# soasme/LTX-Video-GPUPoor

Measured on AMD Instinct MI355X. Metric: denoise-steps/sec + VAE-decode frames/sec, LTX-Video 768x512x97f at 1/8 GPU, higher is better.
Workload: dtype bf16

## Files before the change

include/ltxmi.h:

```cpp
#ifndef LTXMI_H
#define LTXMI_H

#include <stddef.h>
#include <stdint.h>

#ifdef __cplusplus
extern "C" {
#endif

typedef enum ltxmi_status {
    LTXMI_OK = 0,
    LTXMI_ERR_INVALID_ARG = -1,
    LTXMI_ERR_UNSUPPORTED = -2,
    LTXMI_ERR_LAUNCH = -3
} ltxmi_status;

const char* ltxmi_version(void);
const char* ltxmi_last_error(void);
const char* ltxmi_arch(void);

typedef enum ltxmi_epilogue {
    LTXMI_EPI_NONE = 0,
    LTXMI_EPI_GELU_TANH = 1,
    LTXMI_EPI_SILU = 2,
    LTXMI_EPI_GATE_RESIDUAL = 3
} ltxmi_epilogue;

typedef struct ltxmi_gemm_args {
    const void* A;  int64_t lda;
    const void* W;  int64_t ldw;
    const void* bias;
    void*       C;  int64_t ldc;
    int32_t M, N, K;
    int32_t epilogue;
    const void* residual; int64_t ldr;
    const void* gate_table;
    const void* gate_temb;
    int64_t     gate_ld;
    int32_t     rows_per_group;
    int32_t     algo;
    float*      rowsumsq; int32_t rowsumsq_cols; int64_t rowsumsq_ld;
    int32_t     a_kblock; int64_t a_kblock_stride;
} ltxmi_gemm_args;

int ltxmi_gemm_bf16(const ltxmi_gemm_args* args, void* stream);

typedef enum ltxmi_norm_kind { LTXMI_NORM_RMS = 0, LTXMI_NORM_LAYER = 1 } ltxmi_norm_kind;

int ltxmi_norm_modulate_bf16(const void* x, int64_t ldx, void* y, int64_t ldy,
                             int32_t rows, int32_t D, float eps, int32_t kind,
                             const void* scale_table, const void* scale_temb,
                             const void* shift_table, const void* shift_temb,
                             int64_t temb_ld, int32_t rows_per_group, void* stream);

int ltxmi_rmsnorm_rope_bf16(void* x, int64_t ldx, int32_t rows, int32_t D,
                            const void* weight, float eps,
                            const void* cos_tab, const void* sin_tab, int64_t ld_tab,
                            int32_t rope_period, void* stream);
int ltxmi_rmsnorm_rope_rstd_bf16(void* x, int64_t ldx, int32_t rows, int32_t D, const void* weight, float eps,
                                 const void* cos_tab, const void* sin_tab, int64_t ld_tab, int32_t rope_period,
                                 const float* rowsumsq, int64_t rowsumsq_ld, int32_t rowsumsq_blocks,
                                 int32_t norm_dim, float norm_eps, float* rstd_out, void* stream);

typedef struct ltxmi_attn_args {
    const void* q; int64_t q_stride_b, q_stride_l;
    const void* k; int64_t k_stride_b, k_stride_l;
    const void* v; int64_t v_stride_b, v_stride_l;
    void*       o; int64_t o_stride_b, o_stride_l;
    const float* key_bias; int64_t bias_stride_b;
    int32_t B, H, Lq, Lk, head_dim;
    float   softmax_scale;
    const float* q_rowsumsq; int64_t q_rowsumsq_stride_b, q_rowsumsq_stride_l; int32_t q_rowsumsq_blocks;
    const void*  q_norm_weight; float q_norm_eps;
    const void*  rope_cos; const void* rope_sin; int64_t rope_stride_b, rope_stride_l;
    int32_t o_segment_len; int64_t o_stride_segment;
    const float* q_rstd; int64_t q_rstd_stride_b, q_rstd_stride_l;
    uint32_t* redo_counter; int32_t force_exact;
    float* lse; int64_t lse_stride_b, lse_stride_h;
} ltxmi_attn_args;

int ltxmi_attention_fwd_bf16(const ltxmi_attn_args* args, void* stream);
int ltxmi_attention_fuses_qnorm(int32_t B, int32_t H, int32_t Lq, int32_t Lk, int32_t head_dim, int32_t has_key_bias);
int ltxmi_attention_kernel_id(int32_t B, int32_t H, int32_t Lq, int32_t Lk, int32_t head_dim, int32_t has_key_bias,
                              int64_t k_stride_l, int64_t v_stride_l);

#define LTXMI_ATTN_MERGE_MAX 8
typedef struct ltxmi_attn_merge_args {
    int32_t n;
    const void*  o_part[LTXMI_ATTN_MERGE_MAX];   int64_t o_part_stride_b[LTXMI_ATTN_MERGE_MAX], o_part_stride_l[LTXMI_ATTN_MERGE_MAX];
    const float* lse_part[LTXMI_ATTN_MERGE_MAX]; int64_t lse_part_stride_b[LTXMI_ATTN_MERGE_MAX], lse_part_stride_h[LTXMI_ATTN_MERGE_MAX];
    void*  o;   int64_t o_stride_b, o_stride_l;
    float* lse; int64_t lse_stride_b, lse_stride_h;
    int32_t B, H, Lq, head_dim;
} ltxmi_attn_merge_args;
int ltxmi_attention_merge_bf16(const ltxmi_attn_merge_args* args, void* stream);

int ltxmi_rowsumsq_rstd_f32(const float* rowsumsq, int64_t rowsumsq_ld, int32_t rowsumsq_blocks, int32_t rows,
                            int32_t norm_dim, float norm_eps, float* rstd_out, void* stream);

int ltxmi_qkv_norm_rope_pack_bf16(const void* qkv, int64_t ld, int32_t B, int32_t Nl, int32_t D, int32_t P,
                                  const void* q_weight, const void* k_weight, float eps, const void* cos_tab,
                                  const void* sin_tab, int64_t ld_tab, int32_t rope_period, void* out, void* stream);

int ltxmi_silu_bf16(const void* x, void* y, int64_t n, void* stream);
int ltxmi_timestep_embedding_bf16(const float* t, void* out, int32_t n, int32_t dim, void* stream);
int ltxmi_stg_blend_bf16(void* a, int64_t lda, const void* v, int64_t ldv,
                         const float* m, int32_t B, int32_t L, int32_t D, void* stream);
int ltxmi_stg_blend_grouped_bf16(void* a, const void* v, int64_t v_stride_g, int64_t v_stride_b, int64_t v_stride_l,
                                 const float* m, int32_t G, int32_t B, int32_t L, int32_t D, void* stream);

typedef struct ltxmi_conv3d_args {
    const void* x; const void* w; const void* bias; void* y;
    int32_t B, T, H, W, Cin, Cout;
    int32_t causal;
    int32_t pad_replicate;
    int32_t d2s;
    const void* residual;
    int32_t res_channels;
    const void* add;
    int32_t stride_t, stride_hw;
    int32_t tpad, out_T;
    int32_t kernel_t, time_pad_zeros;
    int32_t algo;
    int32_t post_norm;
    const float* post_scale;
    const float* post_shift;
    float post_eps;
    void* y_norm;
    void* workspace; int64_t workspace_bytes;
} ltxmi_conv3d_args;

int ltxmi_conv3d_ndhwc_bf16(const ltxmi_conv3d_args* args, void* stream);
int ltxmi_conv3d_fuses_post_norm(const ltxmi_conv3d_args* args);
int64_t ltxmi_conv3d_workspace_bytes(const ltxmi_conv3d_args* args);

int ltxmi_pixelnorm_ada_silu_bf16(const void* x, void* y, int64_t rows, int32_t C,
                                  int64_t rows_per_batch, const float* scale, const float* shift,
                                  int32_t apply_silu, float eps, void* stream);

int ltxmi_add_bf16(const void* a, const void* b, void* y, int64_t n, void* stream);

int ltxmi_layernorm_affine_bf16(const void* x, void* y, int64_t rows, int32_t C,
                                const void* gamma, const void* beta, float eps, void* stream);

int ltxmi_ncdhw_to_ndhwc_bf16(const void* z, void* y, int32_t B, int32_t C, int32_t T, int32_t H,
                              int32_t W, const float* std, const float* mean, void* stream);
int ltxmi_unpatchify_to_ncdhw_bf16(const void* x, void* y, int32_t B, int32_t T, int32_t H, int32_t W,
                                   int32_t C_out, int32_t patch, void* stream);

int ltxmi_patchify_to_ndhwc_bf16(const void* x, void* y, int32_t B, int32_t C, int32_t T, int32_t H,
                                 int32_t W, int32_t patch, int32_t C_pad, void* stream);
int ltxmi_space_to_depth_skip_bf16(const void* conv, const void* x, void* out, int32_t B, int32_t T,
                                   int32_t H, int32_t W, int32_t Cin, int32_t Cconv, int32_t stride_t,
                                   int32_t stride_hw, int32_t group, void* stream);
int ltxmi_ndhwc_to_ncdhw_bf16(const void* x, int64_t ldx, int32_t c0, void* y, int32_t B, int32_t C,
                              int32_t T, int32_t H, int32_t W, const float* std, const float* mean,
                              void* stream);

#define LTXMI_GUIDANCE_WORKSPACE_FLOATS 2048
int ltxmi_guidance_step_bf16(const void* noise_pred, int64_t n, int32_t num_conds,
                             float guidance_scale, float stg_scale, float rescaling_scale,
                             int32_t do_cfg, int32_t do_stg, int32_t do_rescale,
                             void* latents, int32_t latents_bf16, float dt, float* workspace,
                             void* stream);

int ltxmi_guidance_step_masked_bf16(const void* noise_pred, int64_t n, int32_t num_conds,
                                    float guidance_scale, float stg_scale, float rescaling_scale,
                                    int32_t do_cfg, int32_t do_stg, int32_t do_rescale,
                                    void* latents, int32_t latents_bf16, float dt,
                                    const float* cond_mask, int32_t channels, float t,
                                    float* workspace, void* stream);

int ltxmi_image_cond_noise(void* latents, const void* init_latents, const void* noise, int32_t is_bf16,
                           const float* cond_mask, int64_t tokens, int32_t channels, float noise_scale,
                           float t, void* stream);

int ltxmi_groupnorm_silu_bf16(const void* x, void* y, const void* residual, int32_t samples, int64_t S,
                              int32_t C, int32_t groups, const void* gamma, const void* beta, float eps,
                              float* workspace, void* stream);
int ltxmi_pixel_shuffle2d_ndhwc_bf16(const void* x, void* y, int64_t frames, int32_t H, int32_t W, int32_t C,
                                     void* stream);
int ltxmi_tile_blend(const void* a, void* b, int32_t dtype, int64_t outer, int64_t len_a, int64_t len_b,
                     int64_t inner, int32_t extent, void* stream);
int ltxmi_adain_filter(const void* latents, const void* reference, void* out, int32_t is_bf16, int32_t planes,
                       int64_t n, int64_t n_ref, float factor, void* stream);

#ifdef __cplusplus
}
#endif
#endif
```

ltx-video-gpupoor_amd/csrc/api.hip:

```cpp
#include <stdarg.h>
#include <string.h>

#include "common.h"

namespace ltxmi {

static thread_local char g_err[512] = "";

void set_error(const char* fmt, ...) {
    va_list ap;
    va_start(ap, fmt);
    vsnprintf(g_err, sizeof(g_err), fmt, ap);
    va_end(ap);
}

int check_launch(const char* what) {
    const hipError_t e = hipGetLastError();
    if (e != hipSuccess) {
        set_error("%s: launch failed: %s", what, hipGetErrorString(e));
        return LTXMI_ERR_LAUNCH;
    }
    return LTXMI_OK;
}

int reserve_lds(const void* kernel, int bytes, unsigned long long* done, const char* what) {
    int dev = 0;
    if (hipGetDevice(&dev) != hipSuccess) {
        set_error("%s: cannot query the current device", what);
        return LTXMI_ERR_LAUNCH;
    }
    const bool tracked = dev >= 0 && dev < 64;
    const unsigned long long bit = tracked ? (1ull << dev) : 0ull;
    if (tracked && (__atomic_load_n(done, __ATOMIC_ACQUIRE) & bit)) return LTXMI_OK;
    const hipError_t e = hipFuncSetAttribute(kernel, hipFuncAttributeMaxDynamicSharedMemorySize, bytes);
    if (e != hipSuccess) {
        set_error("%s: cannot reserve %d bytes of LDS: %s", what, bytes, hipGetErrorString(e));
        return LTXMI_ERR_LAUNCH;
    }
    if (tracked) __atomic_fetch_or(done, bit, __ATOMIC_RELEASE);
    return LTXMI_OK;
}

int device_cu_count(const char* what) {
    static int cus[64] = {};
    int dev = 0;
    if (hipGetDevice(&dev) != hipSuccess) {
        set_error("%s: cannot query the current device", what);
        return -1;
    }
    const bool tracked = dev >= 0 && dev < 64;
    if (tracked) {
        const int c = __atomic_load_n(&cus[dev], __ATOMIC_ACQUIRE);
        if (c > 0) return c;
    }
    int n = 0;
    if (hipDeviceGetAttribute(&n, hipDeviceAttributeMultiprocessorCount, dev) != hipSuccess || n <= 0) {
        set_error("%s: cannot query the CU count of device %d", what, dev);
        return -1;
    }
    if (tracked) __atomic_store_n(&cus[dev], n, __ATOMIC_RELEASE);
    return n;
}

}

extern "C" const char* ltxmi_version(void) { return "ltxmi 0.6.0 (round 5)"; }
extern "C" const char* ltxmi_last_error(void) { return ltxmi::g_err; }
extern "C" const char* ltxmi_arch(void) { return "gfx950"; }
```

ltx-video-gpupoor_amd/csrc/attention.h:

```cpp
#pragma once
#include "common.h"

namespace ltxmi {

struct AttnParams {
    const uint16_t* q; int64_t q_sb, q_sl;
    const uint16_t* k; int64_t k_sb, k_sl;
    const uint16_t* v; int64_t v_sb, v_sl;
    uint16_t* o; int64_t o_sb, o_sl;
    const float* bias; int64_t bias_sb;
    int B, H, Lq, Lk;
    float scale_log2e;
    int q_tiles;
    const float* q_ss; int64_t q_ss_sb, q_ss_sl; int q_ss_n;
    const float* q_rstd; int64_t q_rstd_sb, q_rstd_sl;
    const uint16_t* q_w; float q_eps;
    const uint16_t* rope_cos; const uint16_t* rope_sin; int64_t rope_sb, rope_sl;
    int o_seg; int64_t o_sseg;
    uint32_t* redo_count; int force_exact;
    float* lse; int64_t lse_sb, lse_sh;

    __host__ __device__ __forceinline__ bool q_on_load() const { return q_ss != nullptr || q_rstd != nullptr; }
    __device__ __forceinline__ float q_row_rstd(int b, int row, int HD) const {
        if (q_rstd) return q_rstd[(int64_t)b * q_rstd_sb + (int64_t)row * q_rstd_sl];
        const float* ss = q_ss + (int64_t)b * q_ss_sb + (int64_t)row * q_ss_sl;
        float s2 = 0.f;
        if ((q_ss_n & 3) == 0 && (((uintptr_t)ss) & 15) == 0) {
            const f32x4* ss4 = (const f32x4*)ss;
            for (int j = 0; j < (q_ss_n >> 2); ++j) {
                const f32x4 v4 = ss4[j];
                s2 += (v4[0] + v4[1]) + (v4[2] + v4[3]);
            }
        } else {
            for (int j = 0; j < q_ss_n; ++j) s2 += ss[j];
        }
        return rsqrtf(s2 / (float)HD + q_eps);
    }

    __device__ __forceinline__ void store_lse(int b, int head, int row, float m_log2, float l, bool removed) const {
        constexpr float LN2 = 0.6931471805599453f;
        lse[(int64_t)b * lse_sb + (int64_t)head * lse_sh + row] = removed ? -INFINITY : (m_log2 + __log2f(l)) * LN2;
    }

    __device__ __forceinline__ int64_t o_row(int row) const {
        if (o_seg <= 0) return (int64_t)row * o_sl;
        const int sg = row / o_seg;
        return (int64_t)sg * o_sseg + (int64_t)(row - sg * o_seg) * o_sl;
    }
};

enum AttnKernel : int {
    ATTN_DH64 = 0, ATTN_DH64_BIAS = 1, ATTN_DH64_QB2 = 2, ATTN_PIPE = 3,
    ATTN_DH128 = 4, ATTN_DH128_BIAS = 5, ATTN_PIPE128 = 6, ATTN_CROSS = 7,
};
constexpr int ATTN_CROSS_MAX_KEYS = 256;
constexpr float ATTN_BIAS_FLOOR = -1e30f;
constexpr float ATTN_ROW_REMOVED = 0.99f * ATTN_BIAS_FLOOR;

int launch_attn_pipe(AttnParams p, hipStream_t stream);
int launch_attn_pipe128(AttnParams p, hipStream_t stream);
int launch_attn_cross(AttnParams p, hipStream_t stream);

}
```

ltx-video-gpupoor_amd/csrc/attention.hip:

```cpp
#include <type_traits>

#include "attention.h"

namespace ltxmi {

constexpr int KV_TILE = 64;
constexpr int Q_PER_WAVE = 32;
constexpr int Q_PER_WG = 128;
constexpr float LOG2E = 1.4426950408889634f;
constexpr int ATTN_QB_BIG = 2;

template <int DH>
struct AttnCfg {
    static constexpr int ROW_BYTES = DH * 2;
    static constexpr int TILE_BYTES = KV_TILE * DH * 2;
    static constexpr int CHUNKS_PER_ROW = DH / 8;
    static constexpr int LD_PER_THREAD = (KV_TILE * CHUNKS_PER_ROW) / 256;
    static constexpr int KSTEPS = DH / 16;
    static constexpr int DBLK = DH / 32;
    static constexpr int BIAS_BYTES = KV_TILE * 4;
    static constexpr int STAGE_BYTES = 2 * TILE_BYTES + BIAS_BYTES;
    static constexpr int SMEM = 2 * STAGE_BYTES;
    __device__ static __forceinline__ int k_swz(int row) {
        return DH == 64 ? ((row >> 1) & 7) : (row & 15);
    }
};


template <int DH, bool HAS_BIAS, int QB>
__global__ __launch_bounds__(256, (QB == 2 || DH == 128) ? 2 : 1) void attn_fwd_kernel(AttnParams p) {
    using C = AttnCfg<DH>;
    constexpr int QW = Q_PER_WAVE * QB;
    constexpr bool FOLD = !HAS_BIAS && DH == 128;
    extern __shared__ __attribute__((aligned(16))) char smem[];

    const int tid = threadIdx.x;
    const int lane = tid & 63;
    const int wave = __builtin_amdgcn_readfirstlane(tid >> 6);
    const int r = lane & 31;
    const int hh = lane >> 5;

    const int nwg = gridDim.x, orig = blockIdx.x;
    const int xcd = orig & 7, qn = nwg >> 3, rn = nwg & 7;
    const int work = (xcd < rn ? xcd * (qn + 1) : rn * (qn + 1) + (xcd - rn) * qn) + (orig >> 3);
    const int bh = work / p.q_tiles, qt = work % p.q_tiles;
    const int b = bh / p.H, head = bh % p.H;

    const uint16_t* qb = p.q + (int64_t)b * p.q_sb + head * DH;
    const uint16_t* kb_ = p.k + (int64_t)b * p.k_sb + head * DH;
    const uint16_t* vb = p.v + (int64_t)b * p.v_sb + head * DH;
    uint16_t* ob = p.o + (int64_t)b * p.o_sb + head * DH;
    const float* biasb = HAS_BIAS ? p.bias + (int64_t)b * p.bias_sb : nullptr;

    int q_row[QB];
    bf16x8 qf[QB][C::KSTEPS];
#pragma unroll
    for (int i = 0; i < QB; ++i) {
        q_row[i] = qt * (4 * QW) + wave * QW + 32 * i + r;
        const int q_ld = q_row[i] < p.Lq ? q_row[i] : p.Lq - 1;
        const float rstd = p.q_on_load() ? p.q_row_rstd(b, q_ld, p.H * DH) : 0.f;
#pragma unroll
        for (int s = 0; s < C::KSTEPS; ++s) {
            qf[i][s] = *(const bf16x8*)(qb + (int64_t)q_ld * p.q_sl + 16 * s + 8 * hh);
            if (p.q_on_load()) {
                const int col = head * DH + 16 * s + 8 * hh;
                const bf16x8 wv = *(const bf16x8*)(p.q_w + col);
                float o[8];
#pragma unroll
                for (int e = 0; e < 8; ++e) o[e] = (float)qf[i][s][e] * rstd * (float)wv[e];
                if (p.rope_cos) {
                    const int64_t trow = (int64_t)b * p.rope_sb + (int64_t)q_ld * p.rope_sl;
                    const bf16x8 cv = *(const bf16x8*)(p.rope_cos + trow + col), sv = *(const bf16x8*)(p.rope_sin + trow + col);
#pragma unroll
                    for (int e = 0; e < 8; e += 2) {
                        const float r0 = o[e] * (float)cv[e] - o[e + 1] * (float)sv[e];
                        const float r1 = o[e + 1] * (float)cv[e + 1] + o[e] * (float)sv[e + 1];
                        o[e] = r0;
                        o[e + 1] = r1;
                    }
                }
#pragma unroll
                for (int e = 0; e < 8; ++e) qf[i][s][e] = (__bf16)o[e];
            }
            if (FOLD) {
#pragma unroll
                for (int e = 0; e < 8; ++e) qf[i][s][e] = (__bf16)((float)qf[i][s][e] * p.scale_log2e);
            }
        }
    }

    int st_key[C::LD_PER_THREAD], st_koff[C::LD_PER_THREAD], st_voff[C::LD_PER_THREAD], st_col[C::LD_PER_THREAD];
#pragma unroll
    for (int i = 0; i < C::LD_PER_THREAD; ++i) {
        const int c = tid + 256 * i;
        const int key = c / C::CHUNKS_PER_ROW, dc = c % C::CHUNKS_PER_ROW;
        st_key[i] = key;
        st_col[i] = dc * 8;
        st_koff[i] = key * C::ROW_BYTES + ((dc ^ C::k_swz(key)) << 4);
        st_voff[i] = C::TILE_BYTES + ((key >> 3) * C::DBLK + (dc >> 2)) * 512 + (key & 7) * 64 + (dc & 3) * 16;
    }
    u32x4 kreg[C::LD_PER_THREAD], vreg[C::LD_PER_THREAD];
    float breg = 0.f;

    uint32_t k_goff[C::LD_PER_THREAD], v_goff[C::LD_PER_THREAD];
#pragma unroll
    for (int i = 0; i < C::LD_PER_THREAD; ++i) {
        k_goff[i] = (uint32_t)(((int64_t)st_key[i] * p.k_sl + st_col[i]) * 2);
        v_goff[i] = (uint32_t)(((int64_t)st_key[i] * p.v_sl + st_col[i]) * 2);
    }
    auto load_tile = [&](int k0, auto tail_tag) {
        constexpr bool TAIL = decltype(tail_tag)::value;
        if (!TAIL) {
            const char* kt = (const char*)(kb_ + (int64_t)k0 * p.k_sl);
            const char* vt = (const char*)(vb + (int64_t)k0 * p.v_sl);
#pragma unroll
            for (int i = 0; i < C::LD_PER_THREAD; ++i) {
                kreg[i] = *(const u32x4*)(kt + k_goff[i]);
                vreg[i] = *(const u32x4*)(vt + v_goff[i]);
            }
        } else {
#pragma unroll
            for (int i = 0; i < C::LD_PER_THREAD; ++i) {
                int key = k0 + st_key[i];
                key = key < p.Lk ? key : p.Lk - 1;
                kreg[i] = *(const u32x4*)(kb_ + (int64_t)key * p.k_sl + st_col[i]);
                vreg[i] = *(const u32x4*)(vb + (int64_t)key * p.v_sl + st_col[i]);
            }
        }
        if (HAS_BIAS && tid < KV_TILE) {
            const int key = k0 + tid;
            breg = key < p.Lk ? fmaxf(biasb[key] * LOG2E, ATTN_BIAS_FLOOR) : 0.f;
        }
    };
    auto write_tile = [&](int buf) {
        char* s = smem + buf * C::STAGE_BYTES;
#pragma unroll
        for (int i = 0; i < C::LD_PER_THREAD; ++i) {
            *(u32x4*)(s + st_koff[i]) = kreg[i];
            *(u32x4*)(s + st_voff[i]) = vreg[i];
        }
        if (HAS_BIAS && tid < KV_TILE) *(float*)(s + 2 * C::TILE_BYTES + tid * 4) = breg;
    };

    int k_rd[2];
#pragma unroll
    for (int kb = 0; kb < 2; ++kb) k_rd[kb] = (32 * kb + r) * C::ROW_BYTES;
    const int k_sw0 = C::k_swz(r);
    const int g16 = lane >> 4, i16 = lane & 15;
    const int v_rd = C::TILE_BYTES + (4 * (g16 >> 1) + (i16 >> 2)) * 64 + (16 * (g16 & 1) + 4 * (i16 & 3)) * 2;

    f32x16 oT[QB][C::DBLK];
    float m_run[QB];
    f32x4 lT[QB];
    bf16x8 ones;
    {
        const bool on = ((lane & 15) == 0 && ((lane >> 4) & 1) == 0) || ((lane & 15) == 1 && ((lane >> 4) & 1) == 1);
#pragma unroll
        for (int e = 0; e < 8; ++e) ones[e] = on ? (__bf16)1.0f : (__bf16)0.0f;
    }
    bf16x8 kaug, maug[QB];
#pragma unroll
    for (int e = 0; e < 8; ++e) kaug[e] = (hh == 0 && e < 2) ? (__bf16)1.0f : (__bf16)0.0f;
#pragma unroll
    for (int i = 0; i < QB; ++i) {
        m_run[i] = FOLD ? 0.f : -INFINITY;
#pragma unroll
        for (int e = 0; e < 8; ++e) maug[i][e] = (__bf16)0.0f;
        lT[i] = f32x4{0.f, 0.f, 0.f, 0.f};
#pragma unroll
        for (int d = 0; d < C::DBLK; ++d)
#pragma unroll
            for (int e = 0; e < 16; ++e) oT[i][d][e] = 0.f;
    }
    const float c = p.scale_log2e;

    const int nt = (p.Lk + KV_TILE - 1) / KV_TILE;
    const int n_full = p.Lk / KV_TILE;

    auto tile_body = [&](int t, auto tail_tag) {
        constexpr bool TAIL = decltype(tail_tag)::value;
        const int cur = t & 1;
        const char* s = smem + cur * C::STAGE_BYTES;

        f32x16 sT[QB][2];
#pragma unroll
        for (int i = 0; i < QB; ++i)
#pragma unroll
            for (int kb = 0; kb < 2; ++kb) {
#pragma unroll
                for (int e = 0; e < 16; ++e) sT[i][kb][e] = 0.f;
                if (FOLD) sT[i][kb] = __builtin_amdgcn_mfma_f32_32x32x16_bf16(kaug, maug[i], sT[i][kb], 0, 0, 0);
#pragma unroll
                for (int ks = 0; ks < C::KSTEPS; ++ks) {
                    const bf16x8 kf = *(const bf16x8*)(s + k_rd[kb] + (((2 * ks + hh) ^ k_sw0) << 4));
                    sT[i][kb] = __builtin_amdgcn_mfma_f32_32x32x16_bf16(kf, qf[i][ks], sT[i][kb], 0, 0, 0);
                }
            }

#pragma unroll
        for (int i = 0; i < QB; ++i) {
            if (HAS_BIAS) {
                const float* bl = (const float*)(s + 2 * C::TILE_BYTES);
#pragma unroll
                for (int kb = 0; kb < 2; ++kb)
#pragma unroll
                    for (int g = 0; g < 4; ++g) {
                        const f32x4 b4 = *(const f32x4*)(bl + 32 * kb + 8 * g + 4 * hh);
#pragma unroll
                        for (int e = 0; e < 4; ++e)
                            sT[i][kb][4 * g + e] = __builtin_fmaf(sT[i][kb][4 * g + e], c, b4[e]);
                    }
            }
            if (TAIL) {
                const int k0 = t * KV_TILE;
#pragma unroll
                for (int kb = 0; kb < 2; ++kb)
#pragma unroll
                    for (int e = 0; e < 16; ++e) {
                        const int key = k0 + 32 * kb + (e & 3) + 8 * (e >> 2) + 4 * hh;
                        if (key >= p.Lk) sT[i][kb][e] = -INFINITY;
                    }
            }
            float mt;
            {
                auto max3 = [](float a, float b, float c3) { return fmaxf(fmaxf(a, b), c3); };
                float l1[11];
#pragma unroll
                for (int g = 0; g < 5; ++g) {
                    l1[g] = max3(sT[i][0][3 * g], sT[i][0][3 * g + 1], sT[i][0][3 * g + 2]);
                    l1[5 + g] = max3(sT[i][1][3 * g], sT[i][1][3 * g + 1], sT[i][1][3 * g + 2]);
                }
                l1[10] = max3(sT[i][0][15], sT[i][1][15], l1[0]);
                const float a = max3(l1[1], l1[2], l1[3]), b2 = max3(l1[4], l1[5], l1[6]), c2 = max3(l1[7], l1[8], l1[9]);
                mt = fmaxf(max3(a, b2, c2), l1[10]);
            }
            {
                const auto sw = __builtin_amdgcn_permlane32_swap(__float_as_uint(mt), __float_as_uint(mt), false, false);
                mt = fmaxf(__uint_as_float(sw[0]), __uint_as_float(sw[1]));
            }
            float nmoff = 0.f;
            if (FOLD) {
                const bool first = (t == 0);
                if (first || __any(mt > 0.f)) {
                    asm volatile("; max-moved branch (kept a real branch: not if-converted)" ::: "memory");
                    const float dq = (first || mt > 0.f) ? ceilf(mt * 4.0f) * 0.25f : 0.f;
#pragma unroll
                    for (int kb = 0; kb < 2; ++kb)
#pragma unroll
                        for (int e = 0; e < 16; ++e) sT[i][kb][e] -= dq;
                    if (!first) {
                        const float alpha = fast_exp2(-dq);
                        lT[i][0] *= alpha;
                        lT[i][1] *= __shfl(alpha, (lane + 16) & 63, 64);
#pragma unroll
                        for (int d = 0; d < C::DBLK; ++d)
#pragma unroll
                            for (int e = 0; e < 16; ++e) oT[i][d][e] *= alpha;
                    }
                    m_run[i] += dq;
                    const float nm = -m_run[i];
                    const __bf16 mh = (__bf16)nm;
                    const __bf16 ml = (__bf16)(nm - (float)mh);
                    maug[i][0] = hh == 0 ? mh : (__bf16)0.0f;
                    maug[i][1] = hh == 0 ? ml : (__bf16)0.0f;
                }
            } else {
                const float m_new = fmaxf(m_run[i], mt);
                if (__any(m_new != m_run[i])) {
                    asm volatile("; rescale branch (kept a real branch: not if-converted)" ::: "memory");
                    const float alpha = HAS_BIAS ? fast_exp2(m_run[i] - m_new) : fast_exp2((m_run[i] - m_new) * c);
                    lT[i][0] *= alpha;
                    lT[i][1] *= __shfl(alpha, (lane + 16) & 63, 64);
#pragma unroll
                    for (int d = 0; d < C::DBLK; ++d)
#pragma unroll
                        for (int e = 0; e < 16; ++e) oT[i][d][e] *= alpha;
                    m_run[i] = m_new;
                }
                nmoff = HAS_BIAS ? -m_run[i] : -m_run[i] * c;
            }

            bf16x8 pf[4];
#pragma unroll
            for (int kb = 0; kb < 2; ++kb) {
#pragma unroll
                for (int e = 0; e < 16; ++e) {
                    sT[i][kb][e] = fast_exp2(FOLD ? sT[i][kb][e] : (HAS_BIAS ? sT[i][kb][e] + nmoff : __builtin_fmaf(sT[i][kb][e], c, nmoff)));
                }
#pragma unroll
                for (int h2 = 0; h2 < 2; ++h2)
#pragma unroll
                    for (int e = 0; e < 8; ++e) pf[2 * kb + h2][e] = (__bf16)sT[i][kb][8 * h2 + e];
            }

#pragma unroll
            for (int sp = 0; sp < 4; ++sp) {
                lT[i] = __builtin_amdgcn_mfma_f32_16x16x32_bf16(ones, pf[sp], lT[i], 0, 0, 0);
#pragma unroll
                for (int d = 0; d < C::DBLK; ++d) {
                    const char* base = s + v_rd + (2 * sp * C::DBLK + d) * 512;
                    const s16x4 lo = __builtin_amdgcn_ds_read_tr16_b64_v4i16(
                        (__attribute__((address_space(3))) s16x4*)(base));
                    const s16x4 hi = __builtin_amdgcn_ds_read_tr16_b64_v4i16(
                        (__attribute__((address_space(3))) s16x4*)(base + C::DBLK * 512));
                    typedef __attribute__((ext_vector_type(8))) short s16x8;
                    const s16x8 both = __builtin_shufflevector(lo, hi, 0, 1, 2, 3, 4, 5, 6, 7);
                    const bf16x8 vf = __builtin_bit_cast(bf16x8, both);
                    oT[i][d] = __builtin_amdgcn_mfma_f32_32x32x16_bf16(vf, pf[sp], oT[i][d], 0, 0, 0);
                }
            }
        }
    };

    using no_tail = std::integral_constant<bool, false>;
    using with_tail = std::integral_constant<bool, true>;
    if (n_full > 0) load_tile(0, no_tail{}); else load_tile(0, with_tail{});
    write_tile(0);
    __syncthreads();

    for (int t = 0; t < n_full; ++t) {
        const bool has_next = t + 1 < nt;
        if (has_next) {
            if (t + 1 < n_full) load_tile((t + 1) * KV_TILE, no_tail{});
            else load_tile((t + 1) * KV_TILE, with_tail{});
        }
        tile_body(t, no_tail{});
        if (has_next) write_tile((t & 1) ^ 1);
        __syncthreads();
    }
    if (n_full < nt) tile_body(n_full, with_tail{});

#pragma unroll
    for (int i = 0; i < QB; ++i) {
        const float l0 = __shfl(lT[i][0], r & 15, 64), l1 = __shfl(lT[i][1], r & 15, 64);
        const float l = (r & 16) ? l1 : l0;
        const float inv = 1.0f / l;
        if (p.lse != nullptr) {
            const float m2 = (HAS_BIAS || FOLD) ? m_run[i] : m_run[i] * c;
            if (hh == 0 && q_row[i] < p.Lq) p.store_lse(b, head, q_row[i], m2, l, HAS_BIAS && m_run[i] <= ATTN_ROW_REMOVED);
        }
        char* scr = smem + wave * (32 * C::ROW_BYTES);
        if (i == 0) __syncthreads();
#pragma unroll
        for (int d = 0; d < C::DBLK; ++d)
#pragma unroll
            for (int g = 0; g < 4; ++g) {
                u32x2 w;
                w[0] = pack_bf16(oT[i][d][4 * g + 0] * inv, oT[i][d][4 * g + 1] * inv);
                w[1] = pack_bf16(oT[i][d][4 * g + 2] * inv, oT[i][d][4 * g + 3] * inv);
                const int chunk = 4 * d + g;
                *(u32x2*)(scr + r * C::ROW_BYTES + ((chunk ^ (r & 7)) << 4) + hh * 8) = w;
            }
        constexpr int LPR = C::CHUNKS_PER_ROW;
        constexpr int RPI = 64 / LPR;
        const int q0 = qt * (4 * QW) + wave * QW + 32 * i;
#pragma unroll
        for (int t = 0; t < 32 / RPI; ++t) {
            const int row = t * RPI + lane / LPR, chunk = lane % LPR;
            const u32x4 w = *(const u32x4*)(scr + row * C::ROW_BYTES + ((chunk ^ (row & 7)) << 4));
            if (q0 + row < p.Lq) *(u32x4*)(ob + p.o_row(q0 + row) + chunk * 8) = w;
        }
    }
}

template <int DH, bool HAS_BIAS, int QB>
static int launch(AttnParams p, hipStream_t stream) {
    using C = AttnCfg<DH>;
    auto kern = attn_fwd_kernel<DH, HAS_BIAS, QB>;
    static unsigned long long lds_done = 0;
    if (const int rc = reserve_lds((const void*)kern, C::SMEM, &lds_done, "ltxmi_attention_fwd_bf16")) return rc;
    const int q_per_wg = Q_PER_WG * QB;
    p.q_tiles = (p.Lq + q_per_wg - 1) / q_per_wg;
    const int64_t grid = (int64_t)p.B * p.H * p.q_tiles;
    hipLaunchKernelGGL(kern, dim3((unsigned)grid), dim3(256), C::SMEM, stream, p);
    return check_launch("ltxmi_attention_fwd_bf16");
}

static AttnKernel attn_select(int B, int H, int Lq, int Lk, int head_dim, bool has_bias, int64_t k_sl, int64_t v_sl) {
    const int64_t wg256 = (int64_t)B * H * ((Lq + 255) / 256);
    const int64_t rows = (int64_t)Lk + 4 * 64;
    const bool span_ok = (rows * k_sl + head_dim) * 2 < (1ll << 31) && (rows * v_sl + head_dim) * 2 < (1ll << 31);
    if (head_dim == 128) {
        if (!has_bias && wg256 >= 128 && Lk >= 1024 && span_ok) return ATTN_PIPE128;
        return has_bias ? ATTN_DH128_BIAS : ATTN_DH128;
    }
    if (Lk <= ATTN_CROSS_MAX_KEYS && Lq >= 1024) return ATTN_CROSS;
    if (!has_bias && wg256 >= 192 && span_ok) return ATTN_PIPE;
    if (!has_bias && wg256 >= 512) return ATTN_DH64_QB2;
    return has_bias ? ATTN_DH64_BIAS : ATTN_DH64;
}

}

using namespace ltxmi;

extern "C" int ltxmi_attention_fwd_bf16(const ltxmi_attn_args* a, void* stream) {
    LTXMI_REQUIRE(a && a->q && a->k && a->v && a->o, LTXMI_ERR_INVALID_ARG, "ltxmi_attention_fwd_bf16: NULL argument");
    LTXMI_REQUIRE(a->B > 0 && a->H > 0 && a->Lq > 0 && a->Lk > 0, LTXMI_ERR_INVALID_ARG,
                  "ltxmi_attention_fwd_bf16: non-positive shape B=%d H=%d Lq=%d Lk=%d", a->B, a->H, a->Lq, a->Lk);
    LTXMI_REQUIRE(a->head_dim == 64 || a->head_dim == 128, LTXMI_ERR_UNSUPPORTED,
                  "ltxmi_attention_fwd_bf16: head_dim %d not in {64, 128}", a->head_dim);
    const int64_t strides[] = {a->q_stride_b, a->q_stride_l, a->k_stride_b, a->k_stride_l,
                               a->v_stride_b, a->v_stride_l, a->o_stride_b, a->o_stride_l};
    for (int64_t s : strides)
        LTXMI_REQUIRE(s % 8 == 0, LTXMI_ERR_UNSUPPORTED, "ltxmi_attention_fwd_bf16: strides must be multiples of 8 elements");
    LTXMI_REQUIRE((((uintptr_t)a->q | (uintptr_t)a->k | (uintptr_t)a->v | (uintptr_t)a->o) & 15) == 0,
                  LTXMI_ERR_UNSUPPORTED, "ltxmi_attention_fwd_bf16: q/k/v/o must be 16-byte aligned");
    LTXMI_REQUIRE((int64_t)a->B * a->H * ((a->Lq + Q_PER_WG - 1) / Q_PER_WG) < (1ll << 31), LTXMI_ERR_UNSUPPORTED,
                  "ltxmi_attention_fwd_bf16: grid too large");
    AttnParams p;
    p.q = (const uint16_t*)a->q; p.q_sb = a->q_stride_b; p.q_sl = a->q_stride_l;
    p.k = (const uint16_t*)a->k; p.k_sb = a->k_stride_b; p.k_sl = a->k_stride_l;
    p.v = (const uint16_t*)a->v; p.v_sb = a->v_stride_b; p.v_sl = a->v_stride_l;
    p.o = (uint16_t*)a->o; p.o_sb = a->o_stride_b; p.o_sl = a->o_stride_l;
    p.bias = a->key_bias; p.bias_sb = a->bias_stride_b;
    p.B = a->B; p.H = a->H; p.Lq = a->Lq; p.Lk = a->Lk;
    p.scale_log2e = a->softmax_scale * LOG2E;
    p.q_tiles = (a->Lq + Q_PER_WG - 1) / Q_PER_WG;
    p.q_ss = a->q_rowsumsq; p.q_ss_sb = a->q_rowsumsq_stride_b; p.q_ss_sl = a->q_rowsumsq_stride_l;
    p.q_ss_n = a->q_rowsumsq_blocks;
    p.q_rstd = a->q_rstd; p.q_rstd_sb = a->q_rstd_stride_b; p.q_rstd_sl = a->q_rstd_stride_l;
    p.q_w = (const uint16_t*)a->q_norm_weight; p.q_eps = a->q_norm_eps;
    p.rope_cos = (const uint16_t*)a->rope_cos; p.rope_sin = (const uint16_t*)a->rope_sin;
    p.rope_sb = a->rope_stride_b; p.rope_sl = a->rope_stride_l;
    p.o_seg = a->o_segment_len; p.o_sseg = a->o_stride_segment;
    p.redo_count = a->redo_counter; p.force_exact = a->force_exact != 0;
    LTXMI_REQUIRE(a->o_segment_len >= 0 && a->o_stride_segment % 8 == 0, LTXMI_ERR_INVALID_ARG,
                  "ltxmi_attention_fwd_bf16: bad output segment geometry");
    p.lse = a->lse; p.lse_sb = a->lse_stride_b; p.lse_sh = a->lse_stride_h;
    if (a->lse)
        LTXMI_REQUIRE((((uintptr_t)a->lse) & 3) == 0 && a->lse_stride_h >= a->Lq &&
                          (a->B == 1 ? a->lse_stride_b >= 0 : a->lse_stride_b >= (int64_t)a->H * a->lse_stride_h),
                      LTXMI_ERR_INVALID_ARG,
                      "ltxmi_attention_fwd_bf16: lse must be 4-byte aligned with lse_stride_h >= Lq and lse_stride_b >= H * lse_stride_h");
    if (a->q_rowsumsq || a->q_rstd) {
        LTXMI_REQUIRE(a->q_norm_weight && (((uintptr_t)a->q_norm_weight) & 15) == 0 &&
                          (a->q_rstd ? (((uintptr_t)a->q_rstd) & 3) == 0
                                     : (a->q_rowsumsq_blocks == a->H * a->head_dim / 64 && (((uintptr_t)a->q_rowsumsq) & 3) == 0)),
                      LTXMI_ERR_INVALID_ARG, "ltxmi_attention_fwd_bf16: bad q_rowsumsq / q_rstd / q_norm_weight geometry");
        LTXMI_REQUIRE((a->rope_cos == nullptr) == (a->rope_sin == nullptr), LTXMI_ERR_INVALID_ARG,
                      "ltxmi_attention_fwd_bf16: rope_cos and rope_sin must both be given or both be NULL");
        if (a->rope_cos)
            LTXMI_REQUIRE((((uintptr_t)a->rope_cos | (uintptr_t)a->rope_sin) & 15) == 0 && a->rope_stride_l % 8 == 0 &&
                              a->rope_stride_b % 8 == 0,
                          LTXMI_ERR_INVALID_ARG, "ltxmi_attention_fwd_bf16: RoPE tables must be 16-byte aligned rows");
    }
    hipStream_t s = (hipStream_t)stream;
    switch (attn_select(a->B, a->H, a->Lq, a->Lk, a->head_dim, a->key_bias != nullptr, a->k_stride_l, a->v_stride_l)) {
        case ATTN_DH64: return launch<64, false, 1>(p, s);
        case ATTN_DH64_BIAS: return launch<64, true, 1>(p, s);
        case ATTN_DH64_QB2: return launch<64, false, ATTN_QB_BIG>(p, s);
        case ATTN_PIPE: return launch_attn_pipe(p, s);
        case ATTN_DH128: return launch<128, false, 1>(p, s);
        case ATTN_DH128_BIAS: return launch<128, true, 1>(p, s);
        case ATTN_PIPE128: return launch_attn_pipe128(p, s);
        case ATTN_CROSS: return launch_attn_cross(p, s);
    }
}

extern "C" int ltxmi_attention_kernel_id(int32_t B, int32_t H, int32_t Lq, int32_t Lk, int32_t head_dim, int32_t has_key_bias,
                                         int64_t k_stride_l, int64_t v_stride_l) {
    if (B <= 0 || H <= 0 || Lq <= 0 || Lk <= 0 || k_stride_l <= 0 || v_stride_l <= 0) return -1;
    if (head_dim != 64 && head_dim != 128) return -1;
    return attn_select(B, H, Lq, Lk, head_dim, has_key_bias != 0, k_stride_l, v_stride_l);
}

extern "C" int ltxmi_attention_fuses_qnorm(int32_t B, int32_t H, int32_t Lq, int32_t Lk, int32_t head_dim, int32_t has_key_bias) {
    return (B > 0 && H > 0 && Lq > 0 && Lk > 0 && (head_dim == 64 || head_dim == 128) && (H * head_dim) % 64 == 0) ? 1 : 0;
}
```

ltx-video-gpupoor_amd/csrc/attention_cross.hip:

```cpp
#include <type_traits>

#include "attention.h"

namespace ltxmi {

namespace cross {

#ifndef LTXMI_XATTN_STAGGER
#define LTXMI_XATTN_STAGGER 32
#endif

constexpr int DH = 64;
constexpr int KV_TILE = 64;
constexpr int MAX_TILES = 4;
constexpr int ROW_BYTES = DH * 2;
constexpr int TILE_BYTES = KV_TILE * DH * 2;
constexpr int K_OFF = 0, V_OFF = MAX_TILES * TILE_BYTES, BIAS_OFF = 2 * MAX_TILES * TILE_BYTES;
constexpr int SCR_OFF = BIAS_OFF + MAX_TILES * KV_TILE * 16;
constexpr int SCR_BYTES = 32 * 64;
constexpr int QW_OFF = SCR_OFF + 4 * SCR_BYTES;
constexpr int SMEM = QW_OFF + DH * 2;
constexpr int ROWS_PER_IT = 128;
constexpr float LOG2E = 1.4426950408889634f;

__device__ __forceinline__ int k_swz(int row) { return (row >> 1) & 7; }

template <int NT>
__global__ __launch_bounds__(256, 2) void attn_cross_kernel(AttnParams p, int groups, int rows_per_group, int stagger_from) {
    extern __shared__ __attribute__((aligned(16))) char smem[];
    const int tid = threadIdx.x;
    const int lane = tid & 63;
    const int wave = __builtin_amdgcn_readfirstlane(tid >> 6);
    const int r = lane & 31, hh = lane >> 5;

    const int nwg = gridDim.x, orig = blockIdx.x;
    const int xcd = orig & 7, qn = nwg >> 3, rn = nwg & 7;
    const int work = (xcd < rn ? xcd * (qn + 1) : rn * (qn + 1) + (xcd - rn) * qn) + (orig >> 3);
    const int bh = work / groups, grp = work % groups;
    const int b = bh / p.H, head = bh % p.H;
    const int row_begin = grp * rows_per_group;
    const int row_end = min(p.Lq, row_begin + rows_per_group);
    if (row_begin >= row_end) return;
    const int n_it = (row_end - row_begin + ROWS_PER_IT - 1) / ROWS_PER_IT;

    const uint16_t* qb = p.q + (int64_t)b * p.q_sb + head * DH;
    const uint16_t* kb_ = p.k + (int64_t)b * p.k_sb + head * DH;
    const uint16_t* vb = p.v + (int64_t)b * p.v_sb + head * DH;
    uint16_t* ob = p.o + (int64_t)b * p.o_sb + head * DH;
    constexpr int nt = NT;

    {
        u32x4 kreg[NT][2], vreg[NT][2];
#pragma unroll
        for (int t = 0; t < NT; ++t) {
#pragma unroll
                for (int i = 0; i < 2; ++i) {
                    const int c = tid + 256 * i;
                    int key = t * KV_TILE + (c >> 3);
                    key = key < p.Lk ? key : p.Lk - 1;
                    kreg[t][i] = *(const u32x4*)(kb_ + (int64_t)key * p.k_sl + (c & 7) * 8);
                    vreg[t][i] = *(const u32x4*)(vb + (int64_t)key * p.v_sl + (c & 7) * 8);
                }
            }
        if (tid < MAX_TILES * KV_TILE) {
            float bv = ATTN_BIAS_FLOOR;
            if (tid < p.Lk) bv = p.bias ? fmaxf(p.bias[(int64_t)b * p.bias_sb + tid] * (LOG2E / p.scale_log2e), ATTN_BIAS_FLOOR) : 0.f;
            const __bf16 hi = (__bf16)bv;
            const __bf16 lo = (__bf16)(bv - (float)hi);
            u32x4 w = {0u, 0u, 0u, 0u};
            w[0] = (uint32_t)__builtin_bit_cast(uint16_t, hi) | ((uint32_t)__builtin_bit_cast(uint16_t, lo) << 16);
            *(u32x4*)(smem + BIAS_OFF + tid * 16) = w;
        }
#pragma unroll
        for (int t = 0; t < NT; ++t) {
#pragma unroll
                for (int i = 0; i < 2; ++i) {
                    const int c = tid + 256 * i;
                    const int key = c >> 3, dc = c & 7;
                    *(u32x4*)(smem + K_OFF + t * TILE_BYTES + key * ROW_BYTES + ((dc ^ k_swz(key)) << 4)) = kreg[t][i];
                    *(u32x4*)(smem + V_OFF + t * TILE_BYTES + ((key >> 3) * 2 + (dc >> 2)) * 512 + (key & 7) * 64 + (dc & 3) * 16) = vreg[t][i];
                }
            }
    }
    if (p.q_on_load() && tid < 8) *(u32x4*)(smem + QW_OFF + tid * 16) = *(const u32x4*)(p.q_w + head * DH + tid * 8);
    __syncthreads();

    const int k_rd0 = r * ROW_BYTES, k_rd1 = (32 + r) * ROW_BYTES;
    const int k_sw0 = k_swz(r);
    const int g16 = lane >> 4, i16 = lane & 15;
    const int v_rd = (4 * (g16 >> 1) + (i16 >> 2)) * 64 + (16 * (g16 & 1) + 4 * (i16 & 3)) * 2;
    bf16x8 ones;
    {
        const bool on = ((lane & 15) == 0 && ((lane >> 4) & 1) == 0) || ((lane & 15) == 1 && ((lane >> 4) & 1) == 1);
#pragma unroll
        for (int e = 0; e < 8; ++e) ones[e] = on ? (__bf16)1.0f : (__bf16)0.0f;
    }
    const float c = p.scale_log2e;
    char* scr = smem + SCR_OFF + wave * SCR_BYTES;

    bf16x8 qraw[4], qf[4];
    float q_rstd = 0.f;
    int q_ld = 0;
    auto load_q = [&](int it) {
        const int row = row_begin + it * ROWS_PER_IT + wave * 32 + r;
        q_ld = row < p.Lq ? row : p.Lq - 1;
#pragma unroll
        for (int s = 0; s < 4; ++s) qraw[s] = *(const bf16x8*)(qb + (int64_t)q_ld * p.q_sl + 16 * s + 8 * hh);
        if (p.q_on_load()) q_rstd = p.q_row_rstd(b, q_ld, p.H * DH);
    };
    auto finish_q = [&]() {
        if (p.q_on_load()) {
            const int64_t trow = (int64_t)b * p.rope_sb + (int64_t)q_ld * p.rope_sl;
#pragma unroll
            for (int s = 0; s < 4; ++s) {
                const bf16x8 wv = *(const bf16x8*)(smem + QW_OFF + (16 * s + 8 * hh) * 2);
                float o[8];
#pragma unroll
                for (int e = 0; e < 8; ++e) o[e] = (float)qraw[s][e] * q_rstd * (float)wv[e];
                if (p.rope_cos) {
                    const int col = head * DH + 16 * s + 8 * hh;
                    const bf16x8 cv = *(const bf16x8*)(p.rope_cos + trow + col), sv = *(const bf16x8*)(p.rope_sin + trow + col);
#pragma unroll
                    for (int e = 0; e < 8; e += 2) {
                        const float r0 = o[e] * (float)cv[e] - o[e + 1] * (float)sv[e];
                        const float r1 = o[e + 1] * (float)cv[e + 1] + o[e] * (float)sv[e + 1];
                        o[e] = r0;
                        o[e + 1] = r1;
                    }
                }
#pragma unroll
                for (int e = 0; e < 8; ++e) qf[s][e] = (__bf16)o[e];
            }
        } else {
#pragma unroll
            for (int s = 0; s < 4; ++s) qf[s] = qraw[s];
        }
    };
    load_q(0);
    finish_q();
    if (n_it > 1) load_q(1);
    if (blockIdx.x >= (unsigned)stagger_from) __builtin_amdgcn_s_sleep(LTXMI_XATTN_STAGGER);

    for (int it = 0; it < n_it; ++it) {
        const int q0 = row_begin + it * ROWS_PER_IT + wave * 32;

        constexpr int NG = 2 * NT;
        f32x16 sT[NG];
        bf16x8 kfr[5];
        bf16x8 qaug;
        {
            uint32_t w0 = hh == 0 ? 0x3f803f80u : 0u, w1 = 0u;
            asm volatile("" : "+v"(w0), "+v"(w1));
            const u32x4 w = {w0, w1, w1, w1};
            qaug = __builtin_bit_cast(bf16x8, w);
        }
        auto read_k1 = [&](int g, int j) {
            if (j == 0) {
                kfr[0] = *(const bf16x8*)(smem + BIAS_OFF + (32 * g + r) * 16);
            } else {
                const char* ks = smem + K_OFF + (g >> 1) * TILE_BYTES + ((g & 1) ? k_rd1 : k_rd0);
                kfr[j] = *(const bf16x8*)(ks + (((2 * (j - 1) + hh) ^ k_sw0) << 4));
            }
        };
        auto max3 = [](float a, float b2, float c3) { return fmaxf(fmaxf(a, b2), c3); };
        float mt = -INFINITY;
        auto group_max = [&](int g) {
            const f32x16& x = sT[g];
            const float a = max3(x[0], x[1], x[2]), b2 = max3(x[3], x[4], x[5]), c2 = max3(x[6], x[7], x[8]);
            const float d2 = max3(x[9], x[10], x[11]), e2 = max3(x[12], x[13], x[14]);
            mt = max3(max3(a, b2, c2), max3(d2, e2, x[15]), mt);
            asm volatile("" : "+v"(mt));
        };
#pragma unroll
        for (int j = 0; j < 5; ++j) read_k1(0, j);
#pragma unroll
        for (int g = 0; g < NG; ++g) {
#pragma unroll
            for (int j = 0; j < 5; ++j) {
                if (j == 0) {
                    const f32x16 z16 = {0.f, 0.f, 0.f, 0.f, 0.f, 0.f, 0.f, 0.f, 0.f, 0.f, 0.f, 0.f, 0.f, 0.f, 0.f, 0.f};
                    sT[g] = __builtin_amdgcn_mfma_f32_32x32x16_bf16(kfr[0], qaug, z16, 0, 0, 0);
                } else {
                    sT[g] = __builtin_amdgcn_mfma_f32_32x32x16_bf16(kfr[j], qf[j - 1], sT[g], 0, 0, 0);
                }
                if (g + 1 < NG) read_k1(g + 1, j);
                __builtin_amdgcn_sched_barrier(0);
            }
            if (g >= 1) group_max(g - 1);
        }
        if (it + 1 < n_it) finish_q();
        if (it + 2 < n_it) load_q(it + 2);
        group_max(NG - 1);
        {
            const auto sw = __builtin_amdgcn_permlane32_swap(__float_as_uint(mt), __float_as_uint(mt), false, false);
            mt = fmaxf(__uint_as_float(sw[0]), __uint_as_float(sw[1]));
        }
        const float nmc = -mt * c;

        f32x16 oT[2];
        f32x4 lT;
        const f32x16 z16 = {0.f, 0.f, 0.f, 0.f, 0.f, 0.f, 0.f, 0.f, 0.f, 0.f, 0.f, 0.f, 0.f, 0.f, 0.f, 0.f};
        const f32x4 z4 = {0.f, 0.f, 0.f, 0.f};
        typedef __attribute__((ext_vector_type(8))) short s16x8;
        auto read_v = [&](int t, int sp, bf16x8 (&dst)[2]) {
            const char* vs = smem + V_OFF + t * TILE_BYTES + v_rd;
#pragma unroll
            for (int d = 0; d < 2; ++d) {
                const char* base = vs + (2 * sp * 2 + d) * 512;
                const s16x4 lo = __builtin_amdgcn_ds_read_tr16_b64_v4i16((__attribute__((address_space(3))) s16x4*)(base));
                const s16x4 hi = __builtin_amdgcn_ds_read_tr16_b64_v4i16((__attribute__((address_space(3))) s16x4*)(base + 2 * 512));
                const s16x8 both = __builtin_shufflevector(lo, hi, 0, 1, 2, 3, 4, 5, 6, 7);
                dst[d] = __builtin_bit_cast(bf16x8, both);
            }
        };
        auto make_p = [&](int t, int sp2, bf16x8& dst) {
            const f32x16& x = sT[2 * t + (sp2 >> 1)];
            const f32x2 c2v = {c, c}, m2v = {nmc, nmc};
#pragma unroll
            for (int e = 0; e < 8; e += 2) {
                const f32x2 y = f32x2{x[8 * (sp2 & 1) + e], x[8 * (sp2 & 1) + e + 1]} * c2v + m2v;
                dst[e] = (__bf16)fast_exp2(y[0]);
                dst[e + 1] = (__bf16)fast_exp2(y[1]);
            }
            asm volatile("" : "+v"(dst));
        };
        bf16x8 pfr[2][4], vfr[2][2];
#pragma unroll
        for (int sp = 0; sp < 4; ++sp) make_p(0, sp, pfr[0][sp]);
        read_v(0, 0, vfr[0]);
#pragma unroll
        for (int t = 0; t < NT; ++t) {
#pragma unroll
            for (int sp = 0; sp < 4; ++sp) {
                const int st = 4 * t + sp;
                if (st + 1 < 4 * NT) read_v((st + 1) >> 2, (st + 1) & 3, vfr[(st + 1) & 1]);
                const bf16x8& pf = pfr[t & 1][sp];
                lT = __builtin_amdgcn_mfma_f32_16x16x32_bf16(ones, pf, st == 0 ? z4 : lT, 0, 0, 0);
                oT[0] = __builtin_amdgcn_mfma_f32_32x32x16_bf16(vfr[st & 1][0], pf, st == 0 ? z16 : oT[0], 0, 0, 0);
                oT[1] = __builtin_amdgcn_mfma_f32_32x32x16_bf16(vfr[st & 1][1], pf, st == 0 ? z16 : oT[1], 0, 0, 0);
                if (t + 1 < NT) make_p(t + 1, sp, pfr[(t + 1) & 1][sp]);
                __builtin_amdgcn_sched_barrier(0);
            }
        }

        const float l0 = __shfl(lT[0], r & 15, 64), l1v = __shfl(lT[1], r & 15, 64);
        const float lrow = (r & 16) ? l1v : l0;
        const float inv = 1.0f / lrow;
        if (p.lse != nullptr) {
            if (hh == 0 && q0 + r < row_end) p.store_lse(b, head, q0 + r, -nmc, lrow, -nmc / c <= ATTN_ROW_REMOVED);
        }
#pragma unroll
        for (int d = 0; d < 2; ++d) {
#pragma unroll
            for (int g = 0; g < 4; ++g) {
                u32x2 w;
                w[0] = pack_bf16(oT[d][4 * g + 0] * inv, oT[d][4 * g + 1] * inv);
                w[1] = pack_bf16(oT[d][4 * g + 2] * inv, oT[d][4 * g + 3] * inv);
                *(u32x2*)(scr + r * 64 + ((g ^ (r & 3)) << 4) + hh * 8) = w;
            }
#pragma unroll
            for (int t2 = 0; t2 < 2; ++t2) {
                const int row = t2 * 16 + (lane >> 2), chunk = lane & 3;
                const u32x4 w = *(const u32x4*)(scr + row * 64 + ((chunk ^ (row & 3)) << 4));
                if (q0 + row < row_end) *(u32x4*)(ob + p.o_row(q0 + row) + 32 * d + chunk * 8) = w;
            }
        }
    }
}

}

static_assert(cross::MAX_TILES * cross::KV_TILE == ATTN_CROSS_MAX_KEYS, "attn_select hands this kernel up to ATTN_CROSS_MAX_KEYS keys");

int launch_attn_cross(AttnParams p, hipStream_t stream) {
    const int n_cu = device_cu_count("ltxmi_attention_fwd_bf16");
    if (n_cu <= 0) return LTXMI_ERR_LAUNCH;
    const int slots = 2 * n_cu, bh = p.B * p.H;
    int groups = slots / bh;
    if (groups < 1) groups = 1;
    const int max_groups = (p.Lq + 2 * cross::ROWS_PER_IT - 1) / (2 * cross::ROWS_PER_IT);
    if (groups > max_groups) groups = max_groups;
    int rows = (p.Lq + groups - 1) / groups;
    rows = (rows + cross::ROWS_PER_IT - 1) / cross::ROWS_PER_IT * cross::ROWS_PER_IT;
    groups = (p.Lq + rows - 1) / rows;
    const int64_t grid = (int64_t)bh * groups;
    const int nt = (p.Lk + cross::KV_TILE - 1) / cross::KV_TILE;
#define LTXMI_XATTN_LAUNCH(N)                                                                                              \
    {                                                                                                                      \
        static unsigned long long lds_done = 0;                                                                            \
        if (const int rc = reserve_lds((const void*)cross::attn_cross_kernel<N>, cross::SMEM, &lds_done,                   \
                                       "ltxmi_attention_fwd_bf16"))                                                        \
            return rc;                                                                                                     \
        hipLaunchKernelGGL(cross::attn_cross_kernel<N>, dim3((unsigned)grid), dim3(256), cross::SMEM, stream, p, groups,   \
                           rows, n_cu);                                                                                    \
    }
    switch (nt) {
        case 1: LTXMI_XATTN_LAUNCH(1) break;
        case 2: LTXMI_XATTN_LAUNCH(2) break;
        case 3: LTXMI_XATTN_LAUNCH(3) break;
        default: LTXMI_XATTN_LAUNCH(4) break;
    }
#undef LTXMI_XATTN_LAUNCH
    return check_launch("ltxmi_attention_fwd_bf16");
}

}
```

ltx-video-gpupoor_amd/ltxmi/_lib.py:

```python
import ctypes
import os

import torch

_HERE = os.path.dirname(os.path.abspath(__file__))
LIB_PATH = os.environ.get("LTXMI_LIB") or os.path.join(_HERE, "libltxmi.so")

c_void_p, c_int, c_int64, c_float = ctypes.c_void_p, ctypes.c_int32, ctypes.c_int64, ctypes.c_float


class GemmArgs(ctypes.Structure):
    _fields_ = [("A", c_void_p), ("lda", c_int64), ("W", c_void_p), ("ldw", c_int64), ("bias", c_void_p),
                ("C", c_void_p), ("ldc", c_int64), ("M", c_int), ("N", c_int), ("K", c_int),
                ("epilogue", c_int), ("residual", c_void_p), ("ldr", c_int64), ("gate_table", c_void_p),
                ("gate_temb", c_void_p), ("gate_ld", c_int64), ("rows_per_group", c_int), ("algo", c_int),
                ("rowsumsq", c_void_p), ("rowsumsq_cols", c_int), ("rowsumsq_ld", c_int64),
                ("a_kblock", c_int), ("a_kblock_stride", c_int64)]


class AttnArgs(ctypes.Structure):
    _fields_ = [("q", c_void_p), ("q_stride_b", c_int64), ("q_stride_l", c_int64),
                ("k", c_void_p), ("k_stride_b", c_int64), ("k_stride_l", c_int64),
                ("v", c_void_p), ("v_stride_b", c_int64), ("v_stride_l", c_int64),
                ("o", c_void_p), ("o_stride_b", c_int64), ("o_stride_l", c_int64),
                ("key_bias", c_void_p), ("bias_stride_b", c_int64),
                ("B", c_int), ("H", c_int), ("Lq", c_int), ("Lk", c_int), ("head_dim", c_int),
                ("softmax_scale", c_float),
                ("q_rowsumsq", c_void_p), ("q_rowsumsq_stride_b", c_int64), ("q_rowsumsq_stride_l", c_int64),
                ("q_rowsumsq_blocks", c_int), ("q_norm_weight", c_void_p), ("q_norm_eps", c_float),
                ("rope_cos", c_void_p), ("rope_sin", c_void_p), ("rope_stride_b", c_int64), ("rope_stride_l", c_int64),
                ("o_segment_len", c_int), ("o_stride_segment", c_int64),
                ("q_rstd", c_void_p), ("q_rstd_stride_b", c_int64), ("q_rstd_stride_l", c_int64),
                ("redo_counter", c_void_p), ("force_exact", c_int),
                ("lse", c_void_p), ("lse_stride_b", c_int64), ("lse_stride_h", c_int64)]


ATTN_MERGE_MAX = 8


class AttnMergeArgs(ctypes.Structure):
    _fields_ = [("n", c_int),
                ("o_part", c_void_p * ATTN_MERGE_MAX), ("o_part_stride_b", c_int64 * ATTN_MERGE_MAX),
                ("o_part_stride_l", c_int64 * ATTN_MERGE_MAX),
                ("lse_part", c_void_p * ATTN_MERGE_MAX), ("lse_part_stride_b", c_int64 * ATTN_MERGE_MAX),
                ("lse_part_stride_h", c_int64 * ATTN_MERGE_MAX),
                ("o", c_void_p), ("o_stride_b", c_int64), ("o_stride_l", c_int64),
                ("lse", c_void_p), ("lse_stride_b", c_int64), ("lse_stride_h", c_int64),
                ("B", c_int), ("H", c_int), ("Lq", c_int), ("head_dim", c_int)]


class Conv3dArgs(ctypes.Structure):
    _fields_ = [("x", c_void_p), ("w", c_void_p), ("bias", c_void_p), ("y", c_void_p),
                ("B", c_int), ("T", c_int), ("H", c_int), ("W", c_int), ("Cin", c_int), ("Cout", c_int),
                ("causal", c_int), ("pad_replicate", c_int), ("d2s", c_int), ("residual", c_void_p),
                ("res_channels", c_int), ("add", c_void_p),
                ("stride_t", c_int), ("stride_hw", c_int), ("tpad", c_int), ("out_T", c_int),
                ("kernel_t", c_int), ("time_pad_zeros", c_int), ("algo", c_int),
                ("post_norm", c_int), ("post_scale", c_void_p), ("post_shift", c_void_p), ("post_eps", c_float),
                ("y_norm", c_void_p), ("workspace", c_void_p), ("workspace_bytes", c_int64)]


SIGNATURES = {
    "ltxmi_version": (ctypes.c_char_p, []),
    "ltxmi_last_error": (ctypes.c_char_p, []),
    "ltxmi_arch": (ctypes.c_char_p, []),
    "ltxmi_gemm_bf16": (c_int, [ctypes.POINTER(GemmArgs), c_void_p]),
    "ltxmi_norm_modulate_bf16": (c_int, [c_void_p, c_int64, c_void_p, c_int64, c_int, c_int, c_float, c_int,
                                         c_void_p, c_void_p, c_void_p, c_void_p, c_int64, c_int, c_void_p]),
    "ltxmi_rmsnorm_rope_bf16": (c_int, [c_void_p, c_int64, c_int, c_int, c_void_p, c_float, c_void_p, c_void_p,
                                        c_int64, c_int, c_void_p]),
    "ltxmi_rmsnorm_rope_rstd_bf16": (c_int, [c_void_p, c_int64, c_int, c_int, c_void_p, c_float, c_void_p, c_void_p,
                                             c_int64, c_int, c_void_p, c_int64, c_int, c_int, c_float, c_void_p, c_void_p]),
    "ltxmi_rowsumsq_rstd_f32": (c_int, [c_void_p, c_int64, c_int, c_int, c_int, c_float, c_void_p, c_void_p]),
    "ltxmi_qkv_norm_rope_pack_bf16": (c_int, [c_void_p, c_int64, c_int, c_int, c_int, c_int, c_void_p, c_void_p, c_float,
                                              c_void_p, c_void_p, c_int64, c_int, c_void_p, c_void_p]),
    "ltxmi_attention_fwd_bf16": (c_int, [ctypes.POINTER(AttnArgs), c_void_p]),
    "ltxmi_attention_merge_bf16": (c_int, [ctypes.POINTER(AttnMergeArgs), c_void_p]),
    "ltxmi_attention_fuses_qnorm": (c_int, [c_int, c_int, c_int, c_int, c_int, c_int]),
    "ltxmi_attention_kernel_id": (c_int, [c_int, c_int, c_int, c_int, c_int, c_int, c_int64, c_int64]),
    "ltxmi_silu_bf16": (c_int, [c_void_p, c_void_p, c_int64, c_void_p]),
    "ltxmi_timestep_embedding_bf16": (c_int, [c_void_p, c_void_p, c_int, c_int, c_void_p]),
    "ltxmi_stg_blend_bf16": (c_int, [c_void_p, c_int64, c_void_p, c_int64, c_void_p, c_int, c_int, c_int, c_void_p]),
    "ltxmi_stg_blend_grouped_bf16": (c_int, [c_void_p, c_void_p, c_int64, c_int64, c_int64, c_void_p, c_int, c_int, c_int, c_int,
                                             c_void_p]),
    "ltxmi_conv3d_ndhwc_bf16": (c_int, [ctypes.POINTER(Conv3dArgs), c_void_p]),
    "ltxmi_conv3d_fuses_post_norm": (c_int, [ctypes.POINTER(Conv3dArgs)]),
    "ltxmi_conv3d_workspace_bytes": (c_int64, [ctypes.POINTER(Conv3dArgs)]),
    "ltxmi_pixelnorm_ada_silu_bf16": (c_int, [c_void_p, c_void_p, c_int64, c_int, c_int64, c_void_p, c_void_p,
                                              c_int, c_float, c_void_p]),
    "ltxmi_add_bf16": (c_int, [c_void_p, c_void_p, c_void_p, c_int64, c_void_p]),
    "ltxmi_layernorm_affine_bf16": (c_int, [c_void_p, c_void_p, c_int64, c_int, c_void_p, c_void_p, c_float,
                                            c_void_p]),
    "ltxmi_ncdhw_to_ndhwc_bf16": (c_int, [c_void_p, c_void_p, c_int, c_int, c_int, c_int, c_int, c_void_p,
                                          c_void_p, c_void_p]),
    "ltxmi_unpatchify_to_ncdhw_bf16": (c_int, [c_void_p, c_void_p, c_int, c_int, c_int, c_int, c_int, c_int,
                                               c_void_p]),
    "ltxmi_guidance_step_masked_bf16": (c_int, [c_void_p, c_int64, c_int, c_float, c_float, c_float, c_int, c_int,
                                                c_int, c_void_p, c_int, c_float, c_void_p, c_int, c_float, c_void_p,
                                                c_void_p]),
    "ltxmi_image_cond_noise": (c_int, [c_void_p, c_void_p, c_void_p, c_int, c_void_p, c_int64, c_int, c_float,
                                       c_float, c_void_p]),
    "ltxmi_groupnorm_silu_bf16": (c_int, [c_void_p, c_void_p, c_void_p, c_int, c_int64, c_int, c_int, c_void_p,
                                          c_void_p, c_float, c_void_p, c_void_p]),
    "ltxmi_pixel_shuffle2d_ndhwc_bf16": (c_int, [c_void_p, c_void_p, c_int64, c_int, c_int, c_int, c_void_p]),
    "ltxmi_adain_filter": (c_int, [c_void_p, c_void_p, c_void_p, c_int, c_int, c_int64, c_int64, c_float, c_void_p]),
    "ltxmi_tile_blend": (c_int, [c_void_p, c_void_p, c_int, c_int64, c_int64, c_int64, c_int64, c_int, c_void_p]),
    "ltxmi_patchify_to_ndhwc_bf16": (c_int, [c_void_p, c_void_p, c_int, c_int, c_int, c_int, c_int, c_int, c_int,
                                             c_void_p]),
    "ltxmi_space_to_depth_skip_bf16": (c_int, [c_void_p, c_void_p, c_void_p, c_int, c_int, c_int, c_int, c_int,
                                               c_int, c_int, c_int, c_int, c_void_p]),
    "ltxmi_ndhwc_to_ncdhw_bf16": (c_int, [c_void_p, c_int64, c_int, c_void_p, c_int, c_int, c_int, c_int, c_int,
                                          c_void_p, c_void_p, c_void_p]),
    "ltxmi_guidance_step_bf16": (c_int, [c_void_p, c_int64, c_int, c_float, c_float, c_float, c_int, c_int, c_int,
                                         c_void_p, c_int, c_float, c_void_p, c_void_p]),
}


def _load():
    if not os.path.exists(LIB_PATH):
        raise ImportError(
            f"ltxmi: {LIB_PATH} is missing -- build it with `make -C ltx-video-gpupoor_amd/csrc` "
            "(or `python -c 'import __graft_entry__ as g; g.build()'`). There is no fallback path.")
    lib = ctypes.CDLL(LIB_PATH)
    for name, (res, args) in SIGNATURES.items():
        fn = getattr(lib, name)
        fn.restype = res
        fn.argtypes = args
    return lib


lib = _load()


class LtxmiError(RuntimeError):
    pass


def check(status, what):
    if status != 0:
        raise LtxmiError(f"{what} failed ({status}): {lib.ltxmi_last_error().decode()}")
```

ltx-video-gpupoor_amd/ltxmi/attention.py:

```python
from enum import Enum, auto
from typing import Optional

import torch
from torch import nn

from . import ops
from .attention_seam import pay_attention

BF16 = torch.bfloat16


FUSE_CROSS_ATTENTION_Q = True


class SkipLayerStrategy(Enum):
    AttentionSkip = auto()
    AttentionValues = auto()
    Residual = auto()
    TransformerBlock = auto()


def reshape_hidden_states(hidden_states, latent_frames):
    return hidden_states.reshape(hidden_states.shape[0], latent_frames, -1, hidden_states.shape[-1])


def restore_hidden_states_shape(hidden_states):
    return hidden_states.reshape(hidden_states.shape[0], -1, hidden_states.shape[-1])


class RMSNorm(nn.Module):

    def __init__(self, dim, eps: float, elementwise_affine: bool = True):
        super().__init__()
        self.eps = eps
        self.dim = dim
        if elementwise_affine:
            self.weight = nn.Parameter(torch.ones(dim))
        else:
            self.register_parameter("weight", None)


class _NoAffineLayerNorm(nn.Module):
    def __init__(self, dim, eps: float, elementwise_affine: bool = False):
        super().__init__()
        if elementwise_affine:
            raise NotImplementedError("ltxmi: standardisation norms with affine parameters are not on this path")
        self.eps = eps
        self.dim = dim


class GELUProj(nn.Module):

    def __init__(self, dim_in, dim_out, approximate="tanh", bias=True):
        super().__init__()
        self.proj = nn.Linear(dim_in, dim_out, bias=bias)
        self.approximate = approximate


class FeedForward(nn.Module):

    def __init__(self, dim, dim_out=None, mult=4, dropout=0.0, activation_fn="geglu", final_dropout=False,
                 inner_dim=None, bias=True):
        super().__init__()
        if activation_fn != "gelu-approximate":
            raise NotImplementedError(f"ltxmi: activation_fn '{activation_fn}' is not on this path "
                                      "(LTX-Video uses 'gelu-approximate')")
        inner_dim = int(dim * mult) if inner_dim is None else inner_dim
        dim_out = dim if dim_out is None else dim_out
        self.net = nn.ModuleList([GELUProj(dim, inner_dim, "tanh", bias), nn.Dropout(dropout),
                                  nn.Linear(inner_dim, dim_out, bias=bias)])

    def forward(self, hidden_states, scale: float = 1.0):
        h = ops.gemm(hidden_states, self.net[0].proj.weight, self.net[0].proj.bias, epilogue=ops.EPI_GELU_TANH)
        out = ops.gemm(h, self.net[2].weight, self.net[2].bias)
        return out.view(*hidden_states.shape[:-1], out.shape[-1])


class Attention(nn.Module):

    def __init__(self, query_dim, cross_attention_dim=None, heads=8, dim_head=64, dropout=0.0, bias=False,
                 upcast_attention=False, upcast_softmax=False, out_bias=True, scale_qk=True, qk_norm=None,
                 eps=1e-5, rescale_output_factor=1.0, residual_connection=False, processor=None, out_dim=None,
                 use_tpu_flash_attention=False, use_rope=False, **unsupported):
        super().__init__()
        for k, v in unsupported.items():
            if v not in (None, False, 32):
                raise NotImplementedError(f"ltxmi.Attention: argument {k}={v} is not on this path")
        if use_tpu_flash_attention:
            raise NotImplementedError("ltxmi.Attention: TPU flash attention does not exist on MI355X")
        self.inner_dim = out_dim if out_dim is not None else dim_head * heads
        self.query_dim = query_dim
        self.use_bias = bias
        self.is_cross_attention = cross_attention_dim is not None
        self.cross_attention_dim = cross_attention_dim if cross_attention_dim is not None else query_dim
        self.rescale_output_factor = rescale_output_factor
        self.residual_connection = residual_connection
        self.out_dim = out_dim if out_dim is not None else query_dim
        self.use_tpu_flash_attention = False
        self.use_rope = use_rope
        self.scale = dim_head ** -0.5 if scale_qk else 1.0
        self.heads = out_dim // dim_head if out_dim is not None else heads
        if qk_norm is None:
            self.q_norm, self.k_norm = nn.Identity(), nn.Identity()
        elif qk_norm == "rms_norm":
            self.q_norm = RMSNorm(dim_head * heads, eps=1e-5)
            self.k_norm = RMSNorm(dim_head * heads, eps=1e-5)
        else:
            raise NotImplementedError(f"ltxmi.Attention: qk_norm '{qk_norm}' is not on this path")
        self.to_q = nn.Linear(query_dim, self.inner_dim, bias=bias)
        self.to_k = nn.Linear(self.cross_attention_dim, self.inner_dim, bias=bias)
        self.to_v = nn.Linear(self.cross_attention_dim, self.inner_dim, bias=bias)
        self.to_out = nn.ModuleList([nn.Linear(self.inner_dim, self.out_dim, bias=out_bias), nn.Dropout(dropout)])
        self._packs = {}
        self.set_processor(processor if processor is not None else AttnProcessor2_0())

    def set_processor(self, processor) -> None:
        self.processor = processor

    def get_processor(self, return_deprecated_lora: bool = False):
        return self.processor

    def _pack(self, slot, mods):
        srcs = [t for m in mods for t in (m.weight, m.bias) if t is not None]
        key = tuple((t.data_ptr(), ops.tensor_version(t), t.dtype, t.device) for t in srcs)
        hit = self._packs.get(slot)
        if hit is None or hit[0] != key:
            with torch.no_grad():
                w = torch.cat([m.weight for m in mods], dim=0).contiguous()
                b = torch.cat([m.bias for m in mods], dim=0).contiguous() if mods[0].bias is not None else None
            hit = (key, w, b)
            self._packs[slot] = hit
        return hit[1], hit[2]

    def packed_qkv(self):
        if self.cross_attention_dim != self.query_dim:
            raise ValueError("ltxmi.Attention.packed_qkv: query and key/value inputs differ")
        return self._pack("qkv", [self.to_q, self.to_k, self.to_v])

    def packed_kv(self):
        return self._pack("kv", [self.to_k, self.to_v])

    def invalidate_packed(self):
        self._packs = {}
        self.__dict__.pop("_text_kv_cache", None)

    def _load_from_state_dict(self, *a, **k):
        self.invalidate_packed()
        return super()._load_from_state_dict(*a, **k)

    def _apply(self, fn, *a, **k):
        self.invalidate_packed()
        return super()._apply(fn, *a, **k)

    def forward(self, hidden_states, freqs_cis=None, encoder_hidden_states=None, attention_mask=None,
                skip_layer_mask=None, skip_layer_strategy=None, fused_residual=None, **cross_attention_kwargs):
        wrapper = hidden_states if isinstance(hidden_states, list) else [hidden_states]
        return self.processor(self, wrapper, freqs_cis=freqs_cis, encoder_hidden_states=encoder_hidden_states,
                              attention_mask=attention_mask, skip_layer_mask=skip_layer_mask,
                              skip_layer_strategy=skip_layer_strategy, fused_residual=fused_residual)


def _host_mask(mask):
    if mask is None:
        return None
    host = getattr(mask, "_ltxmi_host", None)
    return host if host is not None else [float(x) for x in mask.flatten().tolist()]


class AttnProcessor2_0:

    def attend(self, qkv_list, is_cross, **kw):
        return pay_attention(qkv_list, **kw)

    def __call__(self, attn: Attention, hidden_states_wrapper, freqs_cis, encoder_hidden_states=None,
                 attention_mask=None, temb=None, skip_layer_mask=None, skip_layer_strategy=None,
                 fused_residual=None, *args, **kwargs):
        hidden_states = hidden_states_wrapper[0]
        hidden_states_wrapper.clear()
        if hidden_states.dim() != 3:
            raise NotImplementedError("ltxmi.AttnProcessor2_0: only [B, N, D] inputs are on this path")
        B, N, _ = hidden_states.shape
        D = attn.inner_dim
        H = attn.heads
        dh = D // H
        x2 = hidden_states.reshape(B * N, -1)
        is_cross = encoder_hidden_states is not None
        if is_cross:
            wkv, bkv = attn.packed_kv()
        else:
            wqkv, bqkv = attn.packed_qkv()
        if not isinstance(attn.q_norm, RMSNorm):
            raise NotImplementedError("ltxmi.AttnProcessor2_0: qk_norm=None is not on this path")

        q_fused = None
        if not is_cross:
            fuse_q = ops.attention_fuses_qnorm(B, H, N, N, dh) and D % 64 == 0 and attention_mask is None
            ss = torch.empty((B * N, D // 64), dtype=torch.float32, device=x2.device) if fuse_q else None
            qkv = ops.gemm(x2, wqkv, bqkv, rowsumsq=ss, rowsumsq_cols=D if fuse_q else 0)
            q2, k2, v2 = qkv[:, :D], qkv[:, D:2 * D], qkv[:, 2 * D:]
            cos = sin = None
            period = 0
            if attn.use_rope:
                cos, sin = freqs_cis
                if cos.shape[0] not in (1, B):
                    raise ValueError("freqs_cis batch must be 1 or the batch size")
                cos2, sin2 = cos.reshape(-1, D), sin.reshape(-1, D)
                period = cos2.shape[0]
                cos, sin = cos2, sin2
            if fuse_q:
                rstd = torch.empty((B * N,), dtype=torch.float32, device=x2.device)
                ops.rmsnorm_rope_(k2, attn.k_norm.weight, attn.k_norm.eps, cos, sin, period,
                                  rstd_of=(ss, D, attn.q_norm.eps, rstd))
                q_fused = ((rstd, attn.q_norm.weight, attn.q_norm.eps), (cos, sin, period) if cos is not None else None)
            else:
                ops.rmsnorm_rope_(q2, attn.q_norm.weight, attn.q_norm.eps, cos, sin, period)
                ops.rmsnorm_rope_(k2, attn.k_norm.weight, attn.k_norm.eps, cos, sin, period)
            Lk = N
            q4 = qkv.view(B, N, 3, H, dh)[:, :, 0]
            k4 = qkv.view(B, N, 3, H, dh)[:, :, 1]
            v4 = qkv.view(B, N, 3, H, dh)[:, :, 2]
            v3 = qkv.view(B, N, 3 * D)[:, :, 2 * D:]
        else:
            Bk, Lk, _ = encoder_hidden_states.shape
            fuse_q = FUSE_CROSS_ATTENTION_Q and D % 64 == 0 and bool(ops.attention_fuses_qnorm(B, H, N, Lk, dh, attention_mask is not None))
            ss = torch.empty((B * N, D // 64), dtype=torch.float32, device=x2.device) if fuse_q else None
            q2 = ops.gemm(x2, attn.to_q.weight, attn.to_q.bias, rowsumsq=ss, rowsumsq_cols=D if fuse_q else 0)
            ehs = encoder_hidden_states
            key = (ehs.data_ptr(), tuple(ehs.shape), ops.tensor_version(ehs), wkv.data_ptr(), ops.tensor_version(wkv),
                   attn.k_norm.weight.data_ptr(), ops.tensor_version(attn.k_norm.weight))
            cache = attn.__dict__.setdefault("_text_kv_cache", {})
            hit = cache.get(key) if ops.STEP_INVARIANT_CACHING else None
            if hit is None:
                ready = attn.__dict__.get("_text_kv_ready")
                if ready is not None:
                    full, full_version, kv_full = ready
                    row_bytes = full.stride(0) * full.element_size()
                    off = ehs.data_ptr() - full.data_ptr()
                    if (row_bytes > 0 and off >= 0 and off % row_bytes == 0 and ehs.shape[1:] == full.shape[1:]
                            and off // row_bytes + Bk <= full.shape[0] and ehs.dtype == full.dtype and ehs.is_contiguous()
                            and ops.tensor_version(full) == full_version):
                        r0 = off // row_bytes
                        hit = (kv_full[r0 * Lk:(r0 + Bk) * Lk],)
            if hit is None:
                kv = ops.gemm(ehs.reshape(Bk * Lk, -1), wkv, bkv)
                ops.rmsnorm_rope_(kv[:, :D], attn.k_norm.weight, attn.k_norm.eps)
                if len(cache) >= 4:
                    cache.clear()
                if ops.STEP_INVARIANT_CACHING:
                    cache[key] = (kv, ehs, wkv)
            else:
                kv = hit[0]
            if fuse_q:
                q_fused = ((ops.rowsumsq_rstd(ss, D, attn.q_norm.eps), attn.q_norm.weight, attn.q_norm.eps), None)
            else:
                ops.rmsnorm_rope_(q2, attn.q_norm.weight, attn.q_norm.eps)
            q4 = q2.view(B, N, H, dh)
            k4 = kv.view(Bk, Lk, 2, H, dh)[:, :, 0]
            v4 = kv.view(Bk, Lk, 2, H, dh)[:, :, 1]
            v3 = kv.view(Bk, Lk, 2 * D)[:, :, D:]

        host_mask = _host_mask(skip_layer_mask) if skip_layer_mask is not None else None
        skip_attention = (host_mask is not None and skip_layer_strategy == SkipLayerStrategy.AttentionValues
                          and len(host_mask) == 1 and host_mask[0] == 0)
        if skip_attention:
            a3 = v3.contiguous()
        else:
            mask4 = None
            if attention_mask is not None:
                if attention_mask.dim() != 3 or attention_mask.shape[1] != 1:
                    raise NotImplementedError("ltxmi.AttnProcessor2_0: attention_mask must be a [B,1,Lk] bias")
                mask4 = attention_mask.reshape(B, 1, 1, Lk)
            a4 = self.attend([q4, k4, v4], is_cross, attention_mask=mask4, softmax_scale=attn.scale,
                             q_norm=q_fused[0] if q_fused else None, rope=q_fused[1] if q_fused else None)
            a3 = a4.view(B, N, D)
            if host_mask is not None and any(m != 1.0 for m in host_mask):
                m_dev = skip_layer_mask.reshape(B).to(torch.float32)
                if skip_layer_strategy == SkipLayerStrategy.AttentionValues:
                    ops.stg_blend_(a3, v3, m_dev)
                elif skip_layer_strategy == SkipLayerStrategy.AttentionSkip:
                    ops.stg_blend_(a3, hidden_states, m_dev)

        w_o, b_o = attn.to_out[0].weight, attn.to_out[0].bias
        if fused_residual is not None:
            residual, gate_table, gate_temb, rpg = fused_residual
            ops.gemm(a3.reshape(B * N, D), w_o, b_o, out=residual.reshape(B * N, -1),
                     epilogue=ops.EPI_GATE_RESIDUAL, residual=residual.reshape(B * N, -1),
                     gate_table=gate_table, gate_temb=gate_temb, rows_per_group=rpg)
            return residual
        out = ops.gemm(a3.reshape(B * N, D), w_o, b_o).view(B, N, -1)
        if attn.residual_connection or attn.rescale_output_factor != 1.0:
            raise NotImplementedError("ltxmi.AttnProcessor2_0: residual_connection / rescale_output_factor")
        return out


class BasicTransformerBlock(nn.Module):

    def __init__(self, dim, num_attention_heads, attention_head_dim, dropout=0.0, cross_attention_dim=None,
                 activation_fn="geglu", num_embeds_ada_norm=None, attention_bias=False, only_cross_attention=False,
                 double_self_attention=False, upcast_attention=False, norm_elementwise_affine=True,
                 adaptive_norm="single_scale_shift", standardization_norm="layer_norm", norm_eps=1e-5,
                 qk_norm=None, final_dropout=False, attention_type="default", ff_inner_dim=None, ff_bias=True,
                 attention_out_bias=True, use_tpu_flash_attention=False, use_rope=False):
        super().__init__()
        if adaptive_norm != "single_scale_shift" or only_cross_attention or double_self_attention:
            raise NotImplementedError("ltxmi.BasicTransformerBlock: only the AdaLN-Zero "
                                      "(single_scale_shift) self+cross block is on this path")
        assert standardization_norm in ("layer_norm", "rms_norm")
        self.adaptive_norm = adaptive_norm
        self.norm_kind = ops.NORM_RMS if standardization_norm == "rms_norm" else ops.NORM_LAYER
        make_norm = RMSNorm if standardization_norm == "rms_norm" else _NoAffineLayerNorm
        if norm_elementwise_affine:
            raise NotImplementedError("ltxmi.BasicTransformerBlock: norm_elementwise_affine=True is not on this path")
        self.norm1 = make_norm(dim, eps=norm_eps, elementwise_affine=False)
        self.attn1 = Attention(query_dim=dim, heads=num_attention_heads, dim_head=attention_head_dim,
                               dropout=dropout, bias=attention_bias, cross_attention_dim=None,
                               out_bias=attention_out_bias, qk_norm=qk_norm, use_rope=use_rope)
        if cross_attention_dim is not None:
            self.attn2 = Attention(query_dim=dim, cross_attention_dim=cross_attention_dim,
                                   heads=num_attention_heads, dim_head=attention_head_dim, dropout=dropout,
                                   bias=attention_bias, out_bias=attention_out_bias, qk_norm=qk_norm,
                                   use_rope=use_rope)
        else:
            self.attn2 = None
        self.norm2 = make_norm(dim, norm_eps, False)
        self.ff = FeedForward(dim, dropout=dropout, activation_fn=activation_fn, final_dropout=final_dropout,
                              inner_dim=ff_inner_dim, bias=ff_bias)
        self.scale_shift_table = nn.Parameter(torch.randn(6, dim) / dim ** 0.5)

    def prepare_shared_state(self):
        self.attn1.packed_qkv()
        if self.attn2 is not None:
            self.attn2.packed_kv()

    def forward(self, hidden_states, freqs_cis=None, attention_mask=None, encoder_hidden_states=None,
                encoder_attention_mask=None, timestep=None, cross_attention_kwargs=None, class_labels=None,
                added_cond_kwargs=None, skip_layer_mask=None, skip_layer_strategy: Optional[SkipLayerStrategy] = None):
        if attention_mask is not None:
            raise NotImplementedError("ltxmi.BasicTransformerBlock: a self-attention mask is not on this path")
        B, N, D = hidden_states.shape
        assert timestep.ndim == 3
        T1 = timestep.shape[1]
        if N % T1 != 0:
            raise ValueError(f"per-frame modulation needs tokens ({N}) divisible by frames ({T1})")
        rpg = N // T1
        host_mask = _host_mask(skip_layer_mask)
        if host_mask is not None and min(host_mask) == 1.0:
            skip_layer_mask, host_mask = None, None
        table = self.scale_shift_table
        temb = timestep.reshape(B * T1, 6 * D)
        h2 = hidden_states.view(B * N, D)

        def chunk(i):
            return table[i], temb[:, i * D:(i + 1) * D]

        norm_h = torch.empty_like(hidden_states)
        sc_t, sc_e = chunk(1)
        sh_t, sh_e = chunk(0)
        ops.norm_modulate(h2, norm_h.view(B * N, D), self.norm1.eps, self.norm_kind, sc_t, sc_e, sh_t, sh_e, rpg)
        g_t, g_e = chunk(2)
        self.attn1([norm_h], freqs_cis=freqs_cis, skip_layer_mask=skip_layer_mask,
                   skip_layer_strategy=skip_layer_strategy, fused_residual=(hidden_states, g_t, g_e, rpg))
        del norm_h

        if self.attn2 is not None:
            self.attn2([hidden_states], freqs_cis=freqs_cis, encoder_hidden_states=encoder_hidden_states,
                       attention_mask=encoder_attention_mask, fused_residual=(hidden_states, None, None, 1))

        block_skip = (host_mask is not None and skip_layer_strategy == SkipLayerStrategy.TransformerBlock)
        if block_skip:
            original = hidden_states.clone()

        norm_h = torch.empty_like(hidden_states)
        sc_t, sc_e = chunk(4)
        sh_t, sh_e = chunk(3)
        ops.norm_modulate(h2, norm_h.view(B * N, D), self.norm2.eps, self.norm_kind, sc_t, sc_e, sh_t, sh_e, rpg)
        ff1 = ops.gemm(norm_h.view(B * N, D), self.ff.net[0].proj.weight, self.ff.net[0].proj.bias,
                       epilogue=ops.EPI_GELU_TANH)
        del norm_h
        g_t, g_e = chunk(5)
        ops.gemm(ff1, self.ff.net[2].weight, self.ff.net[2].bias, out=h2, epilogue=ops.EPI_GATE_RESIDUAL,
                 residual=h2, gate_table=g_t, gate_temb=g_e, rows_per_group=rpg)
        del ff1

        if block_skip:
            ops.stg_blend_(hidden_states, original, skip_layer_mask.reshape(B).to(torch.float32))
        return hidden_states
```

ltx-video-gpupoor_amd/ltxmi/attention_seam.py:

```python
import torch

from . import ops


def _key_bias_from_mask(attention_mask, B, Lk):
    m = attention_mask
    if m.dim() != 4 or m.shape[0] != B or m.shape[-1] != Lk:
        raise ValueError(f"pay_attention: attention_mask must be [B, 1|Lq, 1|H, Lk], got {tuple(m.shape)}")
    for d in (1, 2):
        if m.shape[d] != 1 and m.stride(d) != 0:
            raise NotImplementedError(
                "pay_attention: only key biases broadcast over queries and heads are supported "
                f"(mask dim {d} has size {m.shape[d]} with stride {m.stride(d)})")
    key = (m.data_ptr(), tuple(m.shape), tuple(m.stride()), m.dtype, ops.tensor_version(m))
    hit = _BIAS_CACHE.get(key)
    if hit is None:
        if len(_BIAS_CACHE) >= 4:
            _BIAS_CACHE.clear()
        hit = _BIAS_CACHE[key] = (m[:, 0, 0, :].to(torch.float32).contiguous(), m)
    return hit[0]


_BIAS_CACHE = {}


@torch.compiler.disable()
def pay_attention(qkv_list, dropout_p=0., softmax_scale=None, causal=False, window_size=(-1, -1),
                  deterministic=False, version=None, force_attention=None, attention_mask=None,
                  cross_attn=False, q_lens=None, k_lens=None, q_norm=None, rope=None):
    q, k, v = qkv_list
    qkv_list.clear()
    if (q_norm is not None or rope is not None) and (q_lens is not None or k_lens is not None):
        raise NotImplementedError("pay_attention: q_norm / rope on load with q_lens / k_lens")
    if causal or tuple(window_size) != (-1, -1) or dropout_p != 0.:
        raise NotImplementedError("pay_attention: causal / windowed / dropout attention is not on this path")
    if force_attention not in (None, "sdpa"):
        raise NotImplementedError(f"pay_attention: backend '{force_attention}' does not exist here (single HIP backend)")
    out_dtype = q.dtype
    if v.dtype != torch.bfloat16:
        raise TypeError(f"pay_attention: bf16 only on this path, got {v.dtype}")
    q = q.to(v.dtype)
    k = k.to(v.dtype)
    b, lq, lk = q.size(0), q.size(1), k.size(1)
    final_padding = 0

    if b > 1 and k_lens is not None:
        assert attention_mask is None and q_lens is None
        k_lens = [int(x) for x in k_lens]
        chunk_sizes, k_sizes = [], []
        cur, cnt = k_lens[0], 1
        for kl in k_lens[1:]:
            if kl == cur:
                cnt += 1
            else:
                chunk_sizes.append(cnt)
                k_sizes.append(cur)
                cur, cnt = kl, 1
        chunk_sizes.append(cnt)
        k_sizes.append(cur)
        if len(chunk_sizes) > 1 or k_lens[0] != k.shape[1]:
            outs = []
            for sq, sk, sv, sz in zip(torch.split(q, chunk_sizes), torch.split(k, chunk_sizes),
                                      torch.split(v, chunk_sizes), k_sizes):
                outs.append(pay_attention([sq, sk[:, :sz], sv[:, :sz]], softmax_scale=softmax_scale))
            return torch.cat(outs, dim=0)
    elif q_lens is not None or k_lens is not None:
        assert b == 1
        szq = int(q_lens[0]) if q_lens is not None else lq
        szk = int(k_lens[0]) if k_lens is not None else lk
        final_padding = lq - szq
        q, k, v = q[:, :szq], k[:, :szk], v[:, :szk]

    bias = None if attention_mask is None else _key_bias_from_mask(attention_mask, b, k.size(1))
    x = ops.attention(q, k, v, key_bias=bias, softmax_scale=softmax_scale, q_norm=q_norm, rope=rope)
    x = x.type(out_dtype)
    if final_padding > 0:
        x = torch.cat([x, torch.empty((x.shape[0], final_padding, *x.shape[-2:]), dtype=x.dtype, device=x.device)], 1)
    return x
```

ltx-video-gpupoor_amd/ltxmi/ops.py:

```python
import ctypes
import math

import torch

from . import _lib
from ._lib import lib, check

BF16 = torch.bfloat16

EPI_NONE, EPI_GELU_TANH, EPI_SILU, EPI_GATE_RESIDUAL = 0, 1, 2, 3
NORM_RMS, NORM_LAYER = 0, 1


def _stream():
    return ctypes.c_void_p(torch.cuda.current_stream().cuda_stream)


_watch = None
_events = {}


def watch_launches(keys):
    global _watch
    _watch = set(keys) if keys else None
    _events.clear()


_redo_counter = None


def count_attention_redos(counter):
    global _redo_counter
    _redo_counter = counter


def launch_times_ms():
    return {k: [a.elapsed_time(b) for a, b in v] for k, v in _events.items()}


def _prof_begin(key, key2=None):
    if _watch is None:
        return None
    if key not in _watch:
        if key2 is None or key2 not in _watch:
            return None
        key = key2
    e0, e1 = torch.cuda.Event(enable_timing=True), torch.cuda.Event(enable_timing=True)
    e0.record()
    return key, e0, e1


def _prof_end(tok):
    if tok is not None:
        tok[2].record()
        _events.setdefault(tok[0], []).append((tok[1], tok[2]))


def _ptr(t):
    return None if t is None else ctypes.c_void_p(t.data_ptr())


def _chk_bf16(*ts):
    for t in ts:
        if t is None:
            continue
        if t.dtype != BF16 or not t.is_cuda:
            raise TypeError(f"ltxmi: expected a CUDA bfloat16 tensor, got {t.dtype} on {t.device}")


def _rows(t):
    if t.stride(-1) != 1:
        raise ValueError("ltxmi: innermost dimension must be contiguous")
    t2 = t.reshape(-1, t.shape[-1]) if t.is_contiguous() else t
    if t2.dim() != 2:
        raise ValueError("ltxmi: expected a 2-D tensor or a contiguous N-D tensor")
    return t2, t2.shape[0], t2.stride(0)


def tensor_version(t):
    try:
        return t._version
    except RuntimeError:
        return -1


def gemm(a, w, bias=None, out=None, epilogue=EPI_NONE, residual=None, gate_table=None, gate_temb=None,
         rows_per_group=1, algo=0, rowsumsq=None, rowsumsq_cols=0, a_kblock=0, a_kblock_stride=0):
    _chk_bf16(a, w, bias, out, residual, gate_table, gate_temb)
    a2, M, lda = _rows(a)
    N, K = w.shape
    if a_kblock:
        if a2.shape[1] != a_kblock or K % a_kblock:
            raise ValueError(f"ltxmi.gemm: K-blocked a must be [M, {a_kblock}] with K={K} a multiple of the block")
    elif a2.shape[1] != K:
        raise ValueError(f"ltxmi.gemm: a is [{M},{a2.shape[1]}] but w is [{N},{K}]")
    if out is None:
        out = torch.empty((M, N), dtype=BF16, device=a.device)
    o2, Mo, ldc = _rows(out)
    if Mo != M or o2.shape[1] != N:
        raise ValueError("ltxmi.gemm: bad out shape")
    args = _lib.GemmArgs()
    args.A, args.lda = a2.data_ptr(), lda
    args.W, args.ldw = w.data_ptr(), w.stride(0)
    args.bias = bias.data_ptr() if bias is not None else None
    args.C, args.ldc = o2.data_ptr(), ldc
    args.M, args.N, args.K = M, N, K
    args.epilogue = epilogue
    if residual is not None:
        r2, Mr, ldr = _rows(residual)
        args.residual, args.ldr = r2.data_ptr(), ldr
    if gate_table is not None:
        args.gate_table = gate_table.data_ptr()
        args.gate_temb = gate_temb.data_ptr()
        args.gate_ld = gate_temb.stride(0) if gate_temb.dim() == 2 else 0
    args.rows_per_group = rows_per_group
    args.algo = algo
    args.a_kblock, args.a_kblock_stride = a_kblock, a_kblock_stride
    if rowsumsq is not None:
        if rowsumsq.dtype != torch.float32 or rowsumsq.dim() != 2 or rowsumsq.shape[0] != M or rowsumsq.stride(1) != 1 \
                or rowsumsq.shape[1] * 64 < rowsumsq_cols:
            raise ValueError("ltxmi.gemm: rowsumsq must be fp32 [M, >= rowsumsq_cols/64]")
        args.rowsumsq, args.rowsumsq_cols, args.rowsumsq_ld = rowsumsq.data_ptr(), rowsumsq_cols, rowsumsq.stride(0)
    tok = _prof_begin(("gemm", M, N, K, epilogue))
    check(lib.ltxmi_gemm_bf16(ctypes.byref(args), _stream()), "ltxmi_gemm_bf16")
    _prof_end(tok)
    return out


def norm_modulate(x, out, eps, kind, scale_table, scale_temb, shift_table, shift_temb, rows_per_group):
    _chk_bf16(x, out, scale_table, scale_temb, shift_table, shift_temb)
    x2, rows, ldx = _rows(x)
    o2, _, ldy = _rows(out)
    D = x2.shape[1]
    if scale_temb.stride(0) != shift_temb.stride(0):
        raise ValueError("ltxmi.norm_modulate: scale/shift tables must share a row stride")
    check(lib.ltxmi_norm_modulate_bf16(_ptr(x2), ldx, _ptr(o2), ldy, rows, D, eps, kind,
                                       _ptr(scale_table), _ptr(scale_temb), _ptr(shift_table), _ptr(shift_temb),
                                       scale_temb.stride(0), rows_per_group, _stream()),
          "ltxmi_norm_modulate_bf16")
    return out


def rmsnorm_rope_(x, weight, eps, cos=None, sin=None, rope_period=0, rstd_of=None):
    _chk_bf16(x, weight, cos, sin)
    x2, rows, ldx = _rows(x)
    D = x2.shape[1]
    ld_tab = 0
    if cos is not None:
        if cos.dim() != 2 or cos.shape != sin.shape or cos.stride(0) != sin.stride(0):
            raise ValueError("ltxmi.rmsnorm_rope_: cos/sin must be matching 2-D tables")
        ld_tab = cos.stride(0)
        rope_period = rope_period or cos.shape[0]
    if rstd_of is not None:
        ss, norm_dim, norm_eps, out = rstd_of
        if ss.dtype != torch.float32 or out.dtype != torch.float32 or ss.dim() != 2 or ss.shape[0] != rows or \
                ss.stride(1) != 1 or out.shape != (rows,) or not out.is_contiguous():
            raise ValueError("ltxmi.rmsnorm_rope_: rstd_of needs fp32 sums [rows, blocks] and a contiguous fp32 out [rows]")
        check(lib.ltxmi_rmsnorm_rope_rstd_bf16(_ptr(x2), ldx, rows, D, _ptr(weight), eps, _ptr(cos), _ptr(sin), ld_tab,
                                               rope_period, _ptr(ss), ss.stride(0), ss.shape[1], norm_dim, norm_eps,
                                               _ptr(out), _stream()), "ltxmi_rmsnorm_rope_rstd_bf16")
        return x
    check(lib.ltxmi_rmsnorm_rope_bf16(_ptr(x2), ldx, rows, D, _ptr(weight), eps, _ptr(cos), _ptr(sin), ld_tab,
                                      rope_period, _stream()), "ltxmi_rmsnorm_rope_bf16")
    return x


def rowsumsq_rstd(ss, norm_dim, eps, out=None):
    if ss.dtype != torch.float32 or ss.dim() != 2 or ss.stride(1) != 1 or not ss.is_cuda:
        raise ValueError("ltxmi.rowsumsq_rstd: expected CUDA fp32 sums [rows, blocks]")
    rows = ss.shape[0]
    out = torch.empty((rows,), dtype=torch.float32, device=ss.device) if out is None else out
    check(lib.ltxmi_rowsumsq_rstd_f32(_ptr(ss), ss.stride(0), ss.shape[1], rows, norm_dim, eps, _ptr(out), _stream()),
          "ltxmi_rowsumsq_rstd_f32")
    return out


def attention_fuses_qnorm(B, H, Lq, Lk, dh, has_key_bias=False):
    return bool(lib.ltxmi_attention_fuses_qnorm(B, H, Lq, Lk, dh, int(has_key_bias)))


def attention_kernel_id(B, H, Lq, Lk, dh, has_key_bias=False, k_stride_l=None, v_stride_l=None):
    ks = 3 * H * dh if k_stride_l is None else k_stride_l
    vs = ks if v_stride_l is None else v_stride_l
    return int(lib.ltxmi_attention_kernel_id(B, H, Lq, Lk, dh, int(has_key_bias), ks, vs))


def attention(q, k, v, out=None, key_bias=None, softmax_scale=None, q_norm=None, rope=None, out_segments=None,
              redo_counter=None, force_exact=False, return_lse=False, lse=None):
    _chk_bf16(q, k, v, out)
    B, Lq, H, dh = q.shape
    Lk = k.shape[1]
    for t in (q, k, v):
        if t.stride(3) != 1 or t.stride(2) != dh:
            raise ValueError("ltxmi.attention: (heads, head_dim) must be contiguous")
    if out is None:
        if out_segments is not None:
            raise ValueError("ltxmi.attention: out_segments needs an explicit out")
        out = torch.empty((B, Lq, H, dh), dtype=BF16, device=q.device)
    if out.dim() != 4 or out.stride(3) != 1 or out.stride(2) != dh:
        raise ValueError("ltxmi.attention: out must be 4-D with (heads, head_dim) contiguous")
    a = _lib.AttnArgs()
    if out_segments is not None:
        seg_len, seg_stride = out_segments
        if seg_len <= 0 or Lq % seg_len != 0 or tuple(out.shape) != (B, seg_len, H, dh):
            raise ValueError(f"ltxmi.attention: out_segments=({seg_len}, {seg_stride}) needs Lq={Lq} to be a multiple of the "
                             f"segment and out to be segment 0's [B, segment, H, dh] view, got {tuple(out.shape)}")
        a.o_segment_len, a.o_stride_segment = seg_len, seg_stride
    elif tuple(out.shape) != (B, Lq, H, dh):
        raise ValueError(f"ltxmi.attention: out must be [B, Lq, H, dh] = {(B, Lq, H, dh)}, got {tuple(out.shape)}")
    a.q, a.q_stride_b, a.q_stride_l = q.data_ptr(), q.stride(0), q.stride(1)
    a.k, a.k_stride_b, a.k_stride_l = k.data_ptr(), k.stride(0), k.stride(1)
    a.v, a.v_stride_b, a.v_stride_l = v.data_ptr(), v.stride(0), v.stride(1)
    a.o, a.o_stride_b, a.o_stride_l = out.data_ptr(), out.stride(0), out.stride(1)
    if key_bias is not None:
        if key_bias.dtype != torch.float32 or key_bias.shape != (B, Lk) or key_bias.stride(1) != 1:
            raise ValueError("ltxmi.attention: key_bias must be fp32 [B, Lk]")
        a.key_bias, a.bias_stride_b = key_bias.data_ptr(), key_bias.stride(0)
    a.B, a.H, a.Lq, a.Lk, a.head_dim = B, H, Lq, Lk, dh
    a.softmax_scale = softmax_scale if softmax_scale is not None else 1.0 / math.sqrt(dh)
    if q_norm is not None:
        ss, w, eps = q_norm
        nb = H * dh // 64
        _chk_bf16(w)
        if ss.dim() == 1:
            if ss.dtype != torch.float32 or ss.shape != (B * Lq,) or ss.stride(0) != 1 or not ss.is_cuda:
                raise ValueError("ltxmi.attention: q_norm row factors must be a contiguous fp32 [B*Lq]")
            a.q_rstd, a.q_rstd_stride_b, a.q_rstd_stride_l = ss.data_ptr(), Lq, 1
        else:
            if ss.dtype != torch.float32 or ss.dim() != 2 or ss.shape != (B * Lq, nb) or ss.stride(1) != 1:
                raise ValueError("ltxmi.attention: q_norm row sums must be fp32 [B*Lq, H*dh/64]")
            a.q_rowsumsq, a.q_rowsumsq_stride_b, a.q_rowsumsq_stride_l = ss.data_ptr(), Lq * ss.stride(0), ss.stride(0)
            a.q_rowsumsq_blocks = nb
        a.q_norm_weight, a.q_norm_eps = w.data_ptr(), eps
        if rope is not None:
            cos, sin, period = rope
            _chk_bf16(cos, sin)
            if period not in (Lq, B * Lq) or cos.stride(0) != sin.stride(0) or cos.stride(1) != 1:
                raise ValueError("ltxmi.attention: rope tables must be [Lq or B*Lq, H*dh] with one row stride")
            a.rope_cos, a.rope_sin = cos.data_ptr(), sin.data_ptr()
            a.rope_stride_l = cos.stride(0)
            a.rope_stride_b = 0 if period == Lq else Lq * cos.stride(0)
    elif rope is not None:
        raise ValueError("ltxmi.attention: rope needs q_norm")
    if redo_counter is None:
        redo_counter = _redo_counter
    if redo_counter is not None:
        if redo_counter.dtype != torch.int32 or redo_counter.numel() != 1 or not redo_counter.is_cuda:
            raise ValueError("ltxmi.attention: redo_counter must be a CUDA int32 tensor of one element")
        a.redo_counter = redo_counter.data_ptr()
    a.force_exact = int(bool(force_exact))
    if return_lse or lse is not None:
        if lse is None:
            lse = torch.empty((B, H, Lq), dtype=torch.float32, device=q.device)
        _chk_lse(lse, B, H, Lq, "ltxmi.attention: lse")
        a.lse, a.lse_stride_b, a.lse_stride_h = lse.data_ptr(), lse.stride(0), lse.stride(1)
    tok = _prof_begin(("attention", B, H, Lq, Lk, dh))
    check(lib.ltxmi_attention_fwd_bf16(ctypes.byref(a), _stream()), "ltxmi_attention_fwd_bf16")
    _prof_end(tok)
    return (out, lse) if lse is not None else out


def _chk_lse(lse, B, H, Lq, what):
    if lse.dtype != torch.float32 or not lse.is_cuda or tuple(lse.shape) != (B, H, Lq) or lse.stride(2) != 1:
        raise ValueError(f"{what} must be a CUDA fp32 [B, H, Lq] = {(B, H, Lq)} tensor with contiguous tokens")


def attention_merge(outs, lses, out=None, return_lse=False, lse=None):
    n = len(outs)
    if n != len(lses) or not 2 <= n <= _lib.ATTN_MERGE_MAX:
        raise ValueError(f"ltxmi.attention_merge: {n} outputs / {len(lses)} lse tensors, need 2 .. {_lib.ATTN_MERGE_MAX} of each")
    _chk_bf16(*outs, out)
    B, Lq, H, dh = outs[0].shape
    if out is None:
        out = torch.empty((B, Lq, H, dh), dtype=BF16, device=outs[0].device)
    a = _lib.AttnMergeArgs()
    a.n = n
    for i, (o, l) in enumerate(zip(outs, lses)):
        if tuple(o.shape) != (B, Lq, H, dh) or o.stride(3) != 1 or o.stride(2) != dh:
            raise ValueError("ltxmi.attention_merge: partial outputs must be [B, Lq, H, dh] with (heads, head_dim) contiguous")
        _chk_lse(l, B, H, Lq, f"ltxmi.attention_merge: lses[{i}]")
        a.o_part[i], a.o_part_stride_b[i], a.o_part_stride_l[i] = o.data_ptr(), o.stride(0), o.stride(1)
        a.lse_part[i], a.lse_part_stride_b[i], a.lse_part_stride_h[i] = l.data_ptr(), l.stride(0), l.stride(1)
    if tuple(out.shape) != (B, Lq, H, dh) or out.stride(3) != 1 or out.stride(2) != dh:
        raise ValueError("ltxmi.attention_merge: out must be [B, Lq, H, dh] with (heads, head_dim) contiguous")
    a.o, a.o_stride_b, a.o_stride_l = out.data_ptr(), out.stride(0), out.stride(1)
    if return_lse or lse is not None:
        if lse is None:
            lse = torch.empty((B, H, Lq), dtype=torch.float32, device=out.device)
        _chk_lse(lse, B, H, Lq, "ltxmi.attention_merge: lse")
        a.lse, a.lse_stride_b, a.lse_stride_h = lse.data_ptr(), lse.stride(0), lse.stride(1)
    a.B, a.H, a.Lq, a.head_dim = B, H, Lq, dh
    check(lib.ltxmi_attention_merge_bf16(ctypes.byref(a), _stream()), "ltxmi_attention_merge_bf16")
    return (out, lse) if lse is not None else out


def qkv_norm_rope_pack(qkv, B, Nl, D, P, q_weight, k_weight, eps, cos=None, sin=None, rope_period=0, out=None):
    _chk_bf16(qkv, q_weight, k_weight, cos, sin, out)
    x2, rows, ld = _rows(qkv)
    if rows != B * Nl or x2.shape[1] != 3 * D:
        raise ValueError("ltxmi.qkv_norm_rope_pack: qkv must be [B*Nl, 3D]")
    if out is None:
        out = torch.empty((P, Nl, B, 3, D // P), dtype=BF16, device=qkv.device)
    if not out.is_contiguous() or out.numel() != rows * 3 * D:
        raise ValueError("ltxmi.qkv_norm_rope_pack: out must be a contiguous [P, Nl, B, 3, D/P] buffer")
    ld_tab = cos.stride(0) if cos is not None else 0
    check(lib.ltxmi_qkv_norm_rope_pack_bf16(_ptr(x2), ld, B, Nl, D, P, _ptr(q_weight), _ptr(k_weight), eps, _ptr(cos),
                                            _ptr(sin), ld_tab, rope_period, _ptr(out), _stream()),
          "ltxmi_qkv_norm_rope_pack_bf16")
    return out


def stg_blend_grouped_(a, v, m_f32):
    _chk_bf16(a, v)
    G, B, L, Dg = a.shape
    if not a.is_contiguous() or v.dim() != 3 or v.shape[0] != B or v.shape[1] != L or v.shape[2] < G * Dg or v.stride(2) != 1:
        raise ValueError("ltxmi.stg_blend_grouped_: a must be contiguous [G,B,L,Dg], v [B,L,>=G*Dg] with unit channel stride")
    check(lib.ltxmi_stg_blend_grouped_bf16(_ptr(a), _ptr(v), Dg, v.stride(0), v.stride(1), _ptr(m_f32), G, B, L, Dg, _stream()),
          "ltxmi_stg_blend_grouped_bf16")
    return a


def silu(x, out=None):
    _chk_bf16(x, out)
    out = torch.empty_like(x) if out is None else out
    check(lib.ltxmi_silu_bf16(_ptr(x), _ptr(out), x.numel(), _stream()), "ltxmi_silu_bf16")
    return out


def add(a, b, out=None):
    _chk_bf16(a, b, out)
    out = torch.empty_like(a) if out is None else out
    check(lib.ltxmi_add_bf16(_ptr(a), _ptr(b), _ptr(out), a.numel(), _stream()), "ltxmi_add_bf16")
    return out


def timestep_embedding(t_f32, dim=256):
    if t_f32.dtype != torch.float32 or not t_f32.is_cuda or not t_f32.is_contiguous():
        raise TypeError("ltxmi.timestep_embedding: expected a contiguous CUDA fp32 vector")
    out = torch.empty((t_f32.numel(), dim), dtype=BF16, device=t_f32.device)
    check(lib.ltxmi_timestep_embedding_bf16(_ptr(t_f32), _ptr(out), t_f32.numel(), dim, _stream()),
          "ltxmi_timestep_embedding_bf16")
    return out


def stg_blend_(a, v, m_f32):
    _chk_bf16(a, v)
    B, L, D = a.shape
    a2, _, lda = _rows(a)
    v2 = v.reshape(B * L, D) if v.is_contiguous() else v
    if v2.dim() == 3:
        if v2.stride(0) != L * v2.stride(1):
            raise ValueError("ltxmi.stg_blend_: v batch stride must equal L * row stride")
        ldv = v2.stride(1)
    else:
        ldv = v2.stride(0)
    check(lib.ltxmi_stg_blend_bf16(_ptr(a2), lda, _ptr(v2), ldv, _ptr(m_f32), B, L, D, _stream()),
          "ltxmi_stg_blend_bf16")
    return a


CONV_ALGO = 0


CONV_POST_NORM_FUSE = True
CONV_SECOND_OUTPUT_FUSE = True
CONV_SPLIT = True
_conv_workspace = {}


def conv3d(x, w_packed, bias, causal, pad_replicate, d2s=False, residual=None, add=None, out=None,
           stride=(1, 1, 1), tpad=0, out_T=0, kernel_t=3, time_pad_zeros=False, algo=None, post_norm=None, keep_raw=False):
    _chk_bf16(x, w_packed, bias, residual, add, out)
    B, T, H, W, Cin = x.shape
    Cout = w_packed.shape[0]
    if not x.is_contiguous() or not w_packed.is_contiguous():
        raise ValueError("ltxmi.conv3d: x and w must be contiguous")
    st, sh, sw = stride
    if sh != sw:
        raise ValueError("ltxmi.conv3d: height and width strides must be equal")
    front = tpad if tpad > 0 else (2 if causal else 1)
    back = 0 if (tpad > 0 or causal) else 1
    oT = out_T if out_T > 0 else (T + front + back - 3) // st + 1
    if kernel_t == 1:
        oT = T
    if w_packed.shape[1] != 9 * kernel_t * Cin:
        raise ValueError(f"ltxmi.conv3d: packed weight has K={w_packed.shape[1]}, expected {9 * kernel_t * Cin}")
    oH, oW = (H - 1) // sh + 1, (W - 1) // sh + 1
    if out is None:
        if d2s:
            out = torch.empty((B, 2 * T - 1, 2 * H, 2 * W, Cout // 8), dtype=BF16, device=x.device)
        else:
            out = torch.empty((B, oT, oH, oW, Cout), dtype=BF16, device=x.device)
    a = _lib.Conv3dArgs()
    a.x, a.w, a.bias, a.y = x.data_ptr(), w_packed.data_ptr(), (bias.data_ptr() if bias is not None else None), out.data_ptr()
    a.B, a.T, a.H, a.W, a.Cin, a.Cout = B, T, H, W, Cin, Cout
    a.causal, a.pad_replicate, a.d2s = int(causal), int(pad_replicate), int(d2s)
    a.stride_t, a.stride_hw, a.tpad, a.out_T = st, sh, tpad, out_T
    a.kernel_t, a.time_pad_zeros = kernel_t, int(time_pad_zeros)
    a.algo = CONV_ALGO if algo is None else algo
    if residual is not None:
        a.residual, a.res_channels = residual.data_ptr(), residual.shape[-1]
    if add is not None:
        if not add.is_contiguous() or add.shape != (B, oT, oH, oW, Cout):
            raise ValueError("ltxmi.conv3d: `add` must be a contiguous [B,T,H,W,Cout] tensor")
        a.add = add.data_ptr()
    out_norm = None
    if keep_raw and post_norm is None:
        raise ValueError("ltxmi.conv3d: keep_raw is for post_norm")
    if post_norm is not None:
        scale, shift, eps = post_norm
        if (scale is None) != (shift is None) or ((d2s or add is not None) and not keep_raw):
            raise ValueError("ltxmi.conv3d: post_norm needs scale and shift together, and (without keep_raw) the plain store "
                             "without `add`")
        c_norm = Cout // 8 if d2s else Cout
        for t in (scale, shift):
            if t is not None and (t.dtype != torch.float32 or not t.is_contiguous() or t.shape != (B, c_norm) or not t.is_cuda):
                raise ValueError("ltxmi.conv3d: post_norm scale / shift must be contiguous fp32 [B, C] device tensors")
        if keep_raw:
            out_norm = torch.empty_like(out)
        if CONV_SECOND_OUTPUT_FUSE if keep_raw else CONV_POST_NORM_FUSE:
            a.post_norm, a.post_scale, a.post_shift, a.post_eps = 1, _ptr(scale), _ptr(shift), eps
            if keep_raw:
                a.y_norm = out_norm.data_ptr()
    if CONV_SPLIT:
        want = int(lib.ltxmi_conv3d_workspace_bytes(ctypes.byref(a)))
        if want > 0:
            key = (x.device, torch.cuda.current_stream().cuda_stream)
            ws = _conv_workspace.get(key)
            if ws is None or ws.numel() < want:
                if ws is None and len(_conv_workspace) >= 8:
                    _conv_workspace.clear()
                ws = _conv_workspace[key] = torch.empty(want, dtype=torch.uint8, device=x.device)
            a.workspace, a.workspace_bytes = ws.data_ptr(), ws.numel()
    if a.post_norm and not lib.ltxmi_conv3d_fuses_post_norm(ctypes.byref(a)):
        a.post_norm, a.post_scale, a.post_shift, a.post_eps, a.y_norm = 0, None, None, 0.0, None
    second_launch = post_norm if post_norm is not None and not a.post_norm else None
    kind = ("second_output" if a.y_norm else "post_norm") if a.post_norm else ("add" if add is not None else "plain")
    tok = _prof_begin(("conv3d", B * oT * oH * oW, Cin, Cout, int(d2s)), ("conv3d", B * oT * oH * oW, Cin, Cout, int(d2s), kind))
    check(lib.ltxmi_conv3d_ndhwc_bf16(ctypes.byref(a), _stream()), "ltxmi_conv3d_ndhwc_bf16")
    _prof_end(tok)
    if second_launch is not None:
        pixelnorm_ada_silu(out, second_launch[0], second_launch[1], True, second_launch[2], out=out_norm if keep_raw else out)
    return (out, out_norm) if keep_raw else out


def pixelnorm_ada_silu(x, scale=None, shift=None, apply_silu=True, eps=1e-8, out=None):
    _chk_bf16(x, out)
    B, C = x.shape[0], x.shape[-1]
    rows = x.numel() // C
    out = torch.empty_like(x) if out is None else out
    check(lib.ltxmi_pixelnorm_ada_silu_bf16(_ptr(x), _ptr(out), rows, C, rows // B, _ptr(scale), _ptr(shift),
                                            int(apply_silu), eps, _stream()), "ltxmi_pixelnorm_ada_silu_bf16")
    return out


def layernorm_affine(x, gamma, beta, eps, out=None):
    _chk_bf16(x, gamma, beta, out)
    C = x.shape[-1]
    out = torch.empty_like(x) if out is None else out
    check(lib.ltxmi_layernorm_affine_bf16(_ptr(x), _ptr(out), x.numel() // C, C, _ptr(gamma), _ptr(beta), eps,
                                          _stream()), "ltxmi_layernorm_affine_bf16")
    return out


def ncdhw_to_ndhwc(z, std=None, mean=None):
    _chk_bf16(z)
    B, C, T, H, W = z.shape
    out = torch.empty((B, T, H, W, C), dtype=BF16, device=z.device)
    check(lib.ltxmi_ncdhw_to_ndhwc_bf16(_ptr(z.contiguous()), _ptr(out), B, C, T, H, W, _ptr(std), _ptr(mean),
                                        _stream()), "ltxmi_ncdhw_to_ndhwc_bf16")
    return out


def unpatchify_to_ncdhw(x, c_out, patch):
    _chk_bf16(x)
    B, T, H, W, _ = x.shape
    out = torch.empty((B, c_out, T, H * patch, W * patch), dtype=BF16, device=x.device)
    check(lib.ltxmi_unpatchify_to_ncdhw_bf16(_ptr(x), _ptr(out), B, T, H, W, c_out, patch, _stream()),
          "ltxmi_unpatchify_to_ncdhw_bf16")
    return out


def patchify_to_ndhwc(x, patch, c_pad):
    _chk_bf16(x)
    B, C, T, H, W = x.shape
    out = torch.empty((B, T, H // patch, W // patch, c_pad), dtype=BF16, device=x.device)
    check(lib.ltxmi_patchify_to_ndhwc_bf16(_ptr(x.contiguous()), _ptr(out), B, C, T, H, W, patch, c_pad, _stream()),
          "ltxmi_patchify_to_ndhwc_bf16")
    return out


def space_to_depth_skip(conv, x, stride):
    _chk_bf16(conv, x)
    B, T, H, W, Cin = x.shape
    Cc = conv.shape[-1]
    st, s, _ = stride
    Tc = T + 1 if st == 2 else T
    if tuple(conv.shape) != (B, Tc, H, W, Cc) or not conv.is_contiguous() or not x.is_contiguous() or Cin % Cc:
        raise ValueError(f"ltxmi.space_to_depth_skip: conv {tuple(conv.shape)} does not match x {tuple(x.shape)}")
    out = torch.empty((B, Tc // st, H // s, W // s, Cc * st * s * s), dtype=BF16, device=x.device)
    check(lib.ltxmi_space_to_depth_skip_bf16(_ptr(conv), _ptr(x), _ptr(out), B, T, H, W, Cin, Cc, st, s, Cin // Cc,
                                             _stream()), "ltxmi_space_to_depth_skip_bf16")
    return out


def ndhwc_to_ncdhw(x, c0, C, std=None, mean=None):
    _chk_bf16(x)
    B, T, H, W, ld = x.shape
    if not x.is_contiguous():
        raise ValueError("ltxmi.ndhwc_to_ncdhw: x must be contiguous")
    out = torch.empty((B, C, T, H, W), dtype=BF16, device=x.device)
    check(lib.ltxmi_ndhwc_to_ncdhw_bf16(_ptr(x), ld, c0, _ptr(out), B, C, T, H, W, _ptr(std), _ptr(mean), _stream()),
          "ltxmi_ndhwc_to_ncdhw_bf16")
    return out


STEP_INVARIANT_CACHING = True
STACKED_TEXT_KV = True


def set_step_invariant_caching(enabled: bool):
    global STEP_INVARIANT_CACHING
    STEP_INVARIANT_CACHING = bool(enabled)


GUIDANCE_WORKSPACE_FLOATS = 2048


def guidance_step_(noise_pred, latents, dt, guidance_scale, stg_scale, rescaling_scale, do_cfg, do_stg, do_rescale,
                   workspace, cond_mask=None, t=0.0):
    _chk_bf16(noise_pred)
    num_conds = noise_pred.shape[0]
    n = noise_pred[0].numel()
    is_bf16 = latents.dtype == BF16
    if not is_bf16 and latents.dtype != torch.float32:
        raise TypeError("ltxmi.guidance_step_: latents must be fp32 or bf16")
    if not latents.is_contiguous() or latents.numel() != n:
        raise ValueError("ltxmi.guidance_step_: latents must be contiguous and match one chunk of noise_pred")
    if workspace.dtype != torch.float32 or workspace.numel() < GUIDANCE_WORKSPACE_FLOATS:
        raise ValueError(f"ltxmi.guidance_step_: workspace must hold {GUIDANCE_WORKSPACE_FLOATS} fp32 values")
    if cond_mask is None:
        check(lib.ltxmi_guidance_step_bf16(_ptr(noise_pred), n, num_conds, guidance_scale, stg_scale, rescaling_scale,
                                           int(do_cfg), int(do_stg), int(do_rescale), _ptr(latents), int(is_bf16),
                                           float(dt), _ptr(workspace), _stream()), "ltxmi_guidance_step_bf16")
        return latents
    C = noise_pred.shape[-1]
    if cond_mask.dtype != torch.float32 or not cond_mask.is_contiguous() or cond_mask.numel() * C != n:
        raise ValueError("ltxmi.guidance_step_: cond_mask must be contiguous fp32 with one value per token")
    check(lib.ltxmi_guidance_step_masked_bf16(_ptr(noise_pred), n, num_conds, guidance_scale, stg_scale,
                                              rescaling_scale, int(do_cfg), int(do_stg), int(do_rescale),
                                              _ptr(latents), int(is_bf16), float(dt), _ptr(cond_mask), C, float(t),
                                              _ptr(workspace), _stream()), "ltxmi_guidance_step_masked_bf16")
    return latents


def image_cond_noise_(latents, init_latents, noise, cond_mask, noise_scale, t):
    is_bf16 = latents.dtype == BF16
    for x in (latents, init_latents, noise):
        if x.dtype != latents.dtype or x.shape != latents.shape or not x.is_contiguous():
            raise ValueError("ltxmi.image_cond_noise_: latents, init_latents and noise must match and be contiguous")
    if latents.dtype not in (BF16, torch.float32) or cond_mask.dtype != torch.float32 or not cond_mask.is_contiguous():
        raise TypeError("ltxmi.image_cond_noise_: fp32/bf16 latents and a contiguous fp32 mask expected")
    C = latents.shape[-1]
    tokens = latents.numel() // C
    if cond_mask.numel() != tokens:
        raise ValueError("ltxmi.image_cond_noise_: one mask value per token expected")
    check(lib.ltxmi_image_cond_noise(_ptr(latents), _ptr(init_latents), _ptr(noise), int(is_bf16), _ptr(cond_mask),
                                     tokens, C, float(noise_scale), float(t), _stream()), "ltxmi_image_cond_noise")
    return latents


def groupnorm_silu(x, gamma, beta, groups, eps, residual=None, samples=None, out=None):
    _chk_bf16(x, gamma, beta, residual, out)
    if not x.is_contiguous() or (residual is not None and (not residual.is_contiguous() or residual.shape != x.shape)):
        raise ValueError("ltxmi.groupnorm_silu: x / residual must be contiguous and equally shaped")
    C = x.shape[-1]
    samples = x.shape[0] if samples is None else samples
    S = x.numel() // C // samples
    out = torch.empty_like(x) if out is None else out
    ws = torch.empty(samples * (max(1, 2048 // samples) * 2 * C + 2 * groups), dtype=torch.float32, device=x.device)
    check(lib.ltxmi_groupnorm_silu_bf16(_ptr(x), _ptr(out), _ptr(residual), samples, S, C, groups, _ptr(gamma),
                                        _ptr(beta), eps, _ptr(ws), _stream()), "ltxmi_groupnorm_silu_bf16")
    return out


def pixel_shuffle2d(x):
    _chk_bf16(x)
    B, T, H, W, C4 = x.shape
    if not x.is_contiguous() or C4 % 32:
        raise ValueError("ltxmi.pixel_shuffle2d: contiguous input with 4*C channels (C % 8 == 0) expected")
    out = torch.empty((B, T, 2 * H, 2 * W, C4 // 4), dtype=BF16, device=x.device)
    check(lib.ltxmi_pixel_shuffle2d_ndhwc_bf16(_ptr(x), _ptr(out), B * T, H, W, C4 // 4, _stream()),
          "ltxmi_pixel_shuffle2d_ndhwc_bf16")
    return out


def adain_filter(latents, reference, factor=1.0):
    if latents.dtype != reference.dtype or latents.dtype not in (BF16, torch.float32):
        raise TypeError("ltxmi.adain_filter: fp32 or bf16 latents and reference of the same dtype expected")
    if latents.shape[:2] != reference.shape[:2]:
        raise ValueError("ltxmi.adain_filter: batch/channel sizes differ")
    latents, reference = latents.contiguous(), reference.contiguous()
    planes = latents.shape[0] * latents.shape[1]
    out = torch.empty_like(latents)
    check(lib.ltxmi_adain_filter(_ptr(latents), _ptr(reference), _ptr(out), int(latents.dtype == BF16), planes,
                                 latents.numel() // planes, reference.numel() // planes, float(factor), _stream()),
          "ltxmi_adain_filter")
    return out


def tile_blend_(a, b, extent, dim):
    codes = {torch.float32: 0, BF16: 1, torch.float16: 2}
    if a.dtype != b.dtype or b.dtype not in codes:
        raise TypeError("ltxmi.tile_blend_: fp32, bf16 or fp16 tensors of the same dtype expected")
    if not (a.is_contiguous() and b.is_contiguous()):
        raise ValueError("ltxmi.tile_blend_: contiguous tensors expected")
    sa, sb = list(a.shape), list(b.shape)
    if len(sa) != len(sb) or sa[:dim] + sa[dim + 1:] != sb[:dim] + sb[dim + 1:]:
        raise ValueError("ltxmi.tile_blend_: shapes differ off the blended axis")
    extent = min(sa[dim], sb[dim], int(extent))
    if extent <= 0:
        return b
    outer = 1
    for n in sb[:dim]:
        outer *= n
    inner = 1
    for n in sb[dim + 1:]:
        inner *= n
    check(lib.ltxmi_tile_blend(_ptr(a), _ptr(b), codes[b.dtype], outer, sa[dim], sb[dim], inner, extent, _stream()),
          "ltxmi_tile_blend")
    return b
```

ltx-video-gpupoor_amd/ltxmi/transformer3d.py:

```python
import contextlib
import math
from dataclasses import dataclass
from typing import Any, Dict, List, Optional

import torch
from torch import nn

from . import ops
from .attention import BasicTransformerBlock, SkipLayerStrategy

BF16 = torch.bfloat16


@dataclass
class Transformer3DModelOutput:
    sample: torch.Tensor


class _TimestepEmbedder(nn.Module):
    def __init__(self, in_channels, dim):
        super().__init__()
        self.linear_1 = nn.Linear(in_channels, dim)
        self.linear_2 = nn.Linear(dim, dim)


class _CombinedTimestepEmbeddings(nn.Module):
    def __init__(self, dim):
        super().__init__()
        self.timestep_embedder = _TimestepEmbedder(256, dim)

    def forward(self, timestep_f32):
        proj = ops.timestep_embedding(timestep_f32.contiguous(), 256)
        te = self.timestep_embedder
        h = ops.gemm(proj, te.linear_1.weight, te.linear_1.bias, epilogue=ops.EPI_SILU)
        return ops.gemm(h, te.linear_2.weight, te.linear_2.bias)


class AdaLayerNormSingle(nn.Module):
    def __init__(self, embedding_dim, use_additional_conditions=False):
        super().__init__()
        assert not use_additional_conditions
        self.emb = _CombinedTimestepEmbeddings(embedding_dim)
        self.linear = nn.Linear(embedding_dim, 6 * embedding_dim, bias=True)

    def forward(self, timestep_f32):
        emb = self.emb(timestep_f32)
        return ops.gemm(ops.silu(emb), self.linear.weight, self.linear.bias), emb


class PixArtAlphaTextProjection(nn.Module):
    def __init__(self, in_features, hidden_size):
        super().__init__()
        self.linear_1 = nn.Linear(in_features, hidden_size)
        self.linear_2 = nn.Linear(hidden_size, hidden_size)

    def forward(self, caption):
        h = ops.gemm(caption.reshape(-1, caption.shape[-1]), self.linear_1.weight, self.linear_1.bias,
                     epilogue=ops.EPI_GELU_TANH)
        return ops.gemm(h, self.linear_2.weight, self.linear_2.bias)


class _Config(dict):
    __getattr__ = dict.__getitem__


class Transformer3DModel(nn.Module):
    def __init__(self, num_attention_heads: int = 16, attention_head_dim: int = 88,
                 in_channels: Optional[int] = None, out_channels: Optional[int] = None, num_layers: int = 1,
                 dropout: float = 0.0, norm_num_groups: int = 32, cross_attention_dim: Optional[int] = None,
                 attention_bias: bool = False, num_vector_embeds: Optional[int] = None,
                 activation_fn: str = "geglu", num_embeds_ada_norm: Optional[int] = None,
                 use_linear_projection: bool = False, only_cross_attention: bool = False,
                 double_self_attention: bool = False, upcast_attention: bool = False,
                 adaptive_norm: str = "single_scale_shift", standardization_norm: str = "layer_norm",
                 norm_elementwise_affine: bool = True, norm_eps: float = 1e-5, attention_type: str = "default",
                 caption_channels: int = None, use_tpu_flash_attention: bool = False,
                 qk_norm: Optional[str] = None, positional_embedding_type: str = "rope",
                 positional_embedding_theta: Optional[float] = None,
                 positional_embedding_max_pos: Optional[List[int]] = None,
                 timestep_scale_multiplier: Optional[float] = None, causal_temporal_positioning: bool = False,
                 **ignored):
        super().__init__()
        self.config = _Config({k: v for k, v in locals().items() if k not in ("self", "ignored", "__class__")})
        if use_tpu_flash_attention:
            raise NotImplementedError("TPU flash attention does not exist on MI355X")
        if positional_embedding_type != "rope":
            raise ValueError("Absolute positional embedding is no longer supported")
        if positional_embedding_theta is None or positional_embedding_max_pos is None:
            raise ValueError("rope needs positional_embedding_theta and positional_embedding_max_pos")
        self.num_attention_heads = num_attention_heads
        self.attention_head_dim = attention_head_dim
        inner_dim = num_attention_heads * attention_head_dim
        self.inner_dim = inner_dim
        self.in_channels = in_channels
        self.patchify_proj = nn.Linear(in_channels, inner_dim, bias=True)
        self.positional_embedding_theta = positional_embedding_theta
        self.positional_embedding_max_pos = positional_embedding_max_pos
        self.use_rope = True
        self.timestep_scale_multiplier = timestep_scale_multiplier
        self.transformer_blocks = nn.ModuleList([
            BasicTransformerBlock(inner_dim, num_attention_heads, attention_head_dim, dropout=dropout,
                                  cross_attention_dim=cross_attention_dim, activation_fn=activation_fn,
                                  num_embeds_ada_norm=num_embeds_ada_norm, attention_bias=attention_bias,
                                  only_cross_attention=only_cross_attention,
                                  double_self_attention=double_self_attention, upcast_attention=upcast_attention,
                                  adaptive_norm=adaptive_norm, standardization_norm=standardization_norm,
                                  norm_elementwise_affine=norm_elementwise_affine, norm_eps=norm_eps,
                                  attention_type=attention_type, qk_norm=qk_norm, use_rope=True)
            for _ in range(num_layers)])
        self.out_channels = in_channels if out_channels is None else out_channels
        self.scale_shift_table = nn.Parameter(torch.randn(2, inner_dim) / inner_dim ** 0.5)
        self.proj_out = nn.Linear(inner_dim, self.out_channels)
        self.adaln_single = AdaLayerNormSingle(inner_dim, use_additional_conditions=False)
        self.caption_projection = None
        if caption_channels is not None:
            self.caption_projection = PixArtAlphaTextProjection(caption_channels, inner_dim)

    @property
    def dtype(self):
        return self.patchify_proj.weight.dtype

    @property
    def device(self):
        return self.patchify_proj.weight.device

    @classmethod
    def from_config(cls, config):
        return cls(**{k: v for k, v in dict(config).items() if not k.startswith("_")})

    @classmethod
    def from_pretrained(cls, pretrained_model_path, *args, device="cuda", dtype=torch.bfloat16, **kwargs):
        from .loading import load_transformer
        return load_transformer(pretrained_model_path, device=device, dtype=dtype)

    def load_state_dict(self, state_dict: Dict, *args, **kwargs):
        if any(k.startswith("model.diffusion_model.") for k in state_dict.keys()):
            state_dict = {k.replace("model.diffusion_model.", ""): v for k, v in state_dict.items()
                          if k.startswith("model.diffusion_model.")}
        return super().load_state_dict(state_dict, *args, **kwargs)

    def create_skip_layer_mask(self, batch_size: int, num_conds: int, ptb_index: int,
                               skip_block_list: Optional[List[int]] = None):
        if skip_block_list is None or len(skip_block_list) == 0:
            return None
        num_layers = len(self.transformer_blocks)
        host = torch.ones((num_layers, batch_size * num_conds), dtype=torch.float32)
        for block_idx in skip_block_list:
            host[block_idx, ptb_index::num_conds] = 0
        mask = host.to(device=self.device, dtype=self.dtype)
        mask._ltxmi_host_rows = [[float(x) for x in row] for row in host.tolist()]
        return mask

    def get_fractional_positions(self, indices_grid):
        return torch.stack([indices_grid[:, i] / self.positional_embedding_max_pos[i] for i in range(3)], dim=-1)

    def precompute_freqs_cis(self, indices_grid, spacing="exp"):
        if spacing != "exp":
            raise NotImplementedError("only the default 'exp' spacing is on this path")
        dtype = torch.float32
        dim = self.inner_dim
        theta = self.positional_embedding_theta
        frac = self.get_fractional_positions(indices_grid)
        indices = theta ** torch.linspace(math.log(1, theta), math.log(theta, theta), dim // 6,
                                          device=frac.device, dtype=dtype)
        indices = indices.to(dtype=dtype) * math.pi / 2
        freqs = (indices * (frac.unsqueeze(-1) * 2 - 1)).transpose(-1, -2).flatten(2)
        cos_freq = freqs.cos().repeat_interleave(2, dim=-1)
        sin_freq = freqs.sin().repeat_interleave(2, dim=-1)
        if dim % 6 != 0:
            cos_freq = torch.cat([torch.ones_like(cos_freq[:, :, : dim % 6]), cos_freq], dim=-1)
            sin_freq = torch.cat([torch.zeros_like(cos_freq[:, :, : dim % 6]), sin_freq], dim=-1)
        return cos_freq.to(self.dtype).contiguous(), sin_freq.to(self.dtype).contiguous()

    def _stacked_text_kv(self, ehs):
        blocks = [b for b in self.transformer_blocks if getattr(b, "attn2", None) is not None]
        if not blocks or ehs.dim() != 3 or not ehs.is_contiguous():
            return
        packs = [b.attn2.packed_kv() for b in blocks]
        if any(bk is None for _, bk in packs) or len({tuple(w.shape) for w, _ in packs}) != 1:
            return
        key = tuple((w.data_ptr(), ops.tensor_version(w), bk.data_ptr(), ops.tensor_version(bk)) for w, bk in packs)
        st = self.__dict__.get("_stacked_kv_weights")
        if st is None or st[0] != key:
            with torch.no_grad():
                st = (key, torch.cat([w for w, _ in packs], 0).contiguous(), torch.cat([bk for _, bk in packs], 0).contiguous(),
                      packs)
            self.__dict__["_stacked_kv_weights"] = st
        _, w_all, b_all, _ = st
        Bk, Lk, _ = ehs.shape
        two_d = packs[0][0].shape[0]
        kv_all = ops.gemm(ehs.reshape(Bk * Lk, -1), w_all, b_all)
        for i, b in enumerate(blocks):
            kv = kv_all[:, i * two_d:(i + 1) * two_d]
            ops.rmsnorm_rope_(kv[:, :two_d // 2], b.attn2.k_norm.weight, b.attn2.k_norm.eps)
            b.attn2.__dict__["_text_kv_ready"] = (ehs, ops.tensor_version(ehs), kv)

    def _run_blocks_microbatched(self, hidden_states, slices, freqs_cis, attention_mask, encoder_hidden_states,
                                 encoder_attention_mask, temb, cross_attention_kwargs, class_labels, layer_mask,
                                 skip_layer_strategy, ltxv_model):
        B = hidden_states.shape[0]
        on_gpu = hidden_states.is_cuda
        streams = None
        for block in self.transformer_blocks:
            block.prepare_shared_state()
        if on_gpu:
            main = torch.cuda.current_stream()
            key = (hidden_states.device, len(slices))
            pool = self.__dict__.setdefault("_mb_streams", {})
            streams = pool.get(key)
            if streams is None:
                streams = pool[key] = [torch.cuda.Stream(device=hidden_states.device) for _ in slices]
            for st in streams:
                st.wait_stream(main)

        def rows(t, sl):
            return t if (t is None or t.shape[0] != B) else t[sl]

        interrupted = False
        for block_idx, block in enumerate(self.transformer_blocks):
            for i, sl in enumerate(slices):
                ctx = torch.cuda.stream(streams[i]) if on_gpu else contextlib.nullcontext()
                with ctx:
                    block(hidden_states[sl], freqs_cis=tuple(rows(t, sl) for t in freqs_cis), attention_mask=attention_mask,
                          encoder_hidden_states=rows(encoder_hidden_states, sl),
                          encoder_attention_mask=rows(encoder_attention_mask, sl), timestep=temb[sl],
                          cross_attention_kwargs=cross_attention_kwargs, class_labels=class_labels,
                          skip_layer_mask=layer_mask(block_idx, sl), skip_layer_strategy=skip_layer_strategy)
            if ltxv_model is not None and ltxv_model._interrupt:
                interrupted = True
                break
        if on_gpu:
            for st in streams:
                main.wait_stream(st)
        return interrupted

    def forward(self, hidden_states: torch.Tensor, freqs_cis: list,
                encoder_hidden_states: Optional[torch.Tensor] = None, timestep: Optional[torch.Tensor] = None,
                class_labels: Optional[torch.LongTensor] = None, cross_attention_kwargs: Dict[str, Any] = None,
                attention_mask: Optional[torch.Tensor] = None, encoder_attention_mask: Optional[torch.Tensor] = None,
                skip_layer_mask: Optional[torch.Tensor] = None,
                skip_layer_strategy: Optional[SkipLayerStrategy] = None, latent_shape=None, joint_pass=True,
                ltxv_model=None, mixed=False, return_dict: bool = True, stg_alias_blocks: int = 0,
                _microbatches=None):
        if self.dtype != BF16:
            raise TypeError("ltxmi.Transformer3DModel runs in bfloat16 only: call .to(torch.bfloat16)")
        if mixed:
            raise NotImplementedError("mixed (fp32 residual stream) precision is not on this path")
        if attention_mask is not None:
            raise NotImplementedError("a self-attention mask is not on this path")
        dtype = self.dtype
        hidden_states = hidden_states.to(dtype)
        B, N, _ = hidden_states.shape
        D = self.inner_dim

        if encoder_attention_mask is not None and encoder_attention_mask.ndim == 2:
            encoder_attention_mask = ((1 - encoder_attention_mask.to(dtype)) * -10000.0).unsqueeze(1)

        hidden_states = ops.gemm(hidden_states.reshape(B * N, -1), self.patchify_proj.weight,
                                 self.patchify_proj.bias).view(B, N, D)

        timestep = timestep.to(torch.float32)
        if self.timestep_scale_multiplier:
            timestep = self.timestep_scale_multiplier * timestep
        if timestep.shape[-1] > 1:
            timestep = timestep.reshape(timestep.shape[0], -1, latent_shape[-2] * latent_shape[-1])[:, :, 0]
        temb, embedded_timestep = self.adaln_single(timestep.flatten())
        temb = temb.view(B, -1, 6 * D)
        embedded_timestep = embedded_timestep.view(B, -1, D)

        if self.caption_projection is not None:
            ehs = encoder_hidden_states
            cp = self.caption_projection
            key = (ehs.data_ptr(), tuple(ehs.shape), ehs.dtype, ops.tensor_version(ehs), cp.linear_1.weight.data_ptr(),
                   ops.tensor_version(cp.linear_1.weight), cp.linear_2.weight.data_ptr(), ops.tensor_version(cp.linear_2.weight))
            cache = self.__dict__.setdefault("_caption_cache", {})
            hit = cache.get(key) if ops.STEP_INVARIANT_CACHING else None
            if hit is None:
                if len(cache) >= 4:
                    cache.clear()
                hit = (cp(ehs.to(dtype)).view(B, -1, D), ehs)
                if ops.STEP_INVARIANT_CACHING:
                    cache[key] = hit
            encoder_hidden_states = hit[0]

        if joint_pass and ops.STACKED_TEXT_KV and not ops.STEP_INVARIANT_CACHING and encoder_hidden_states is not None:
            self._stacked_text_kv(encoder_hidden_states)

        host_rows = None
        if skip_layer_mask is not None:
            host_rows = getattr(skip_layer_mask, "_ltxmi_host_rows", None)
            if host_rows is None:
                host_rows = [[float(x) for x in row] for row in skip_layer_mask.float().cpu().tolist()]

        def layer_mask(block_idx, sl=None):
            if skip_layer_mask is None:
                return None
            m = skip_layer_mask[block_idx] if sl is None else skip_layer_mask[block_idx, sl]
            rows = host_rows[block_idx]
            m._ltxmi_host = rows if sl is None else rows[sl]
            return m

        first_block = 0
        if joint_pass and stg_alias_blocks and B >= 2:
            heads, dh = self.num_attention_heads, self.attention_head_dim
            if ops.attention_kernel_id(B, heads, N, N, dh) != ops.attention_kernel_id(B - 1, heads, N, N, dh):
                stg_alias_blocks = 0
        if joint_pass and stg_alias_blocks and B >= 2:
            first_block = min(int(stg_alias_blocks), len(self.transformer_blocks))
            keep = slice(0, B - 1)
            hs = hidden_states[keep]
            for block_idx in range(first_block):
                self.transformer_blocks[block_idx](
                    hs, freqs_cis=freqs_cis, attention_mask=attention_mask,
                    encoder_hidden_states=encoder_hidden_states[keep],
                    encoder_attention_mask=None if encoder_attention_mask is None else encoder_attention_mask[keep],
                    timestep=temb[keep], cross_attention_kwargs=cross_attention_kwargs, class_labels=class_labels,
                    skip_layer_mask=layer_mask(block_idx, keep), skip_layer_strategy=skip_layer_strategy)
                if ltxv_model is not None and ltxv_model._interrupt:
                    return [None]
            hidden_states[B - 1].copy_(hidden_states[B - 2])
        if joint_pass and _microbatches and len(_microbatches) > 1 and first_block == 0:
            if self._run_blocks_microbatched(hidden_states, _microbatches, freqs_cis, attention_mask, encoder_hidden_states,
                                             encoder_attention_mask, temb, cross_attention_kwargs, class_labels,
                                             layer_mask, skip_layer_strategy, ltxv_model):
                return [None]
        elif joint_pass:
            for block_idx, block in enumerate(self.transformer_blocks):
                if block_idx < first_block:
                    continue
                hidden_states = block(hidden_states, freqs_cis=freqs_cis, attention_mask=attention_mask,
                                      encoder_hidden_states=encoder_hidden_states,
                                      encoder_attention_mask=encoder_attention_mask, timestep=temb,
                                      cross_attention_kwargs=cross_attention_kwargs, class_labels=class_labels,
                                      skip_layer_mask=layer_mask(block_idx),
                                      skip_layer_strategy=skip_layer_strategy)
                if ltxv_model is not None and ltxv_model._interrupt:
                    return [None]
        else:
            for block_idx, block in enumerate(self.transformer_blocks):
                for i in range(B):
                    block(hidden_states[i:i + 1], freqs_cis=freqs_cis, attention_mask=attention_mask,
                          encoder_hidden_states=encoder_hidden_states[i:i + 1],
                          encoder_attention_mask=encoder_attention_mask[i:i + 1], timestep=temb[i:i + 1],
                          cross_attention_kwargs=cross_attention_kwargs, class_labels=class_labels,
                          skip_layer_mask=layer_mask(block_idx, slice(i, i + 1)),
                          skip_layer_strategy=skip_layer_strategy)
                    if ltxv_model is not None and ltxv_model._interrupt:
                        return [None]

        for block in self.transformer_blocks:
            if getattr(block, "attn2", None) is not None:
                block.attn2.__dict__.pop("_text_kv_ready", None)

        T1 = embedded_timestep.shape[1]
        emb2 = embedded_timestep.reshape(B * T1, D)
        normed = torch.empty_like(hidden_states)
        ops.norm_modulate(hidden_states.view(B * N, D), normed.view(B * N, D), 1e-6, ops.NORM_LAYER,
                          self.scale_shift_table[1], emb2, self.scale_shift_table[0], emb2, N // T1)
        out = ops.gemm(normed.view(B * N, D), self.proj_out.weight, self.proj_out.bias).view(B, N, -1)
        if not return_dict:
            return (out,)
        return Transformer3DModelOutput(sample=out)
```

Baseline: 16.38.

## Skip padded text key tiles in cross-attention via per-batch valid key counts

Computes, from the encoder attention mask, the last non-padded text token per batch item and passes it to the attention kernels as a valid_keys array. The cross-attention kernel dispatches on this count to a smaller tile-count specialization, so key/value tiles made only of padding are not loaded or computed. The general kernel treats keys past the count as masked. This aims to cut cross-attention work when prompts are shorter than the padded text length. It adds a per-step mask reduction, per-block handover state, and more kernel instantiations.

```diff
diff --git a/include/ltxmi.h b/include/ltxmi.h
--- a/include/ltxmi.h
+++ b/include/ltxmi.h
@@ -68,6 +68,7 @@
     const void* v; int64_t v_stride_b, v_stride_l;
     void*       o; int64_t o_stride_b, o_stride_l;
     const float* key_bias; int64_t bias_stride_b;
+    const int32_t* valid_keys;
     int32_t B, H, Lq, Lk, head_dim;
     float   softmax_scale;
     const float* q_rowsumsq; int64_t q_rowsumsq_stride_b, q_rowsumsq_stride_l; int32_t q_rowsumsq_blocks;
diff --git a/ltx-video-gpupoor_amd/csrc/api.hip b/ltx-video-gpupoor_amd/csrc/api.hip
--- a/ltx-video-gpupoor_amd/csrc/api.hip
+++ b/ltx-video-gpupoor_amd/csrc/api.hip
@@ -64,6 +64,6 @@
 
 }
 
-extern "C" const char* ltxmi_version(void) { return "ltxmi 0.6.0 (round 5)"; }
+extern "C" const char* ltxmi_version(void) { return "ltxmi 0.7.0 (round 5)"; }
 extern "C" const char* ltxmi_last_error(void) { return ltxmi::g_err; }
 extern "C" const char* ltxmi_arch(void) { return "gfx950"; }
diff --git a/ltx-video-gpupoor_amd/csrc/attention.h b/ltx-video-gpupoor_amd/csrc/attention.h
--- a/ltx-video-gpupoor_amd/csrc/attention.h
+++ b/ltx-video-gpupoor_amd/csrc/attention.h
@@ -19,6 +19,7 @@
     int o_seg; int64_t o_sseg;
     uint32_t* redo_count; int force_exact;
     float* lse; int64_t lse_sb, lse_sh;
+    const int32_t* valid_keys;
 
     __host__ __device__ __forceinline__ bool q_on_load() const { return q_ss != nullptr || q_rstd != nullptr; }
     __device__ __forceinline__ float q_row_rstd(int b, int row, int HD) const {
diff --git a/ltx-video-gpupoor_amd/csrc/attention.hip b/ltx-video-gpupoor_amd/csrc/attention.hip
--- a/ltx-video-gpupoor_amd/csrc/attention.hip
+++ b/ltx-video-gpupoor_amd/csrc/attention.hip
@@ -50,7 +50,8 @@
     const uint16_t* kb_ = p.k + (int64_t)b * p.k_sb + head * DH;
     const uint16_t* vb = p.v + (int64_t)b * p.v_sb + head * DH;
     uint16_t* ob = p.o + (int64_t)b * p.o_sb + head * DH;
-    const float* biasb = HAS_BIAS ? p.bias + (int64_t)b * p.bias_sb : nullptr;
+    const float* biasb = HAS_BIAS && p.bias ? p.bias + (int64_t)b * p.bias_sb : nullptr;
+    const int lk_valid = HAS_BIAS && p.valid_keys ? min(p.valid_keys[b], p.Lk) : p.Lk;
 
     int q_row[QB];
     bf16x8 qf[QB][C::KSTEPS];
@@ -129,7 +130,7 @@
         }
         if (HAS_BIAS && tid < KV_TILE) {
             const int key = k0 + tid;
-            breg = key < p.Lk ? fmaxf(biasb[key] * LOG2E, ATTN_BIAS_FLOOR) : 0.f;
+            breg = key < lk_valid ? (biasb ? fmaxf(biasb[key] * LOG2E, ATTN_BIAS_FLOOR) : 0.f) : (key < p.Lk ? ATTN_BIAS_FLOOR : 0.f);
         }
     };
     auto write_tile = [&](int buf) {
@@ -414,6 +415,8 @@
     p.v = (const uint16_t*)a->v; p.v_sb = a->v_stride_b; p.v_sl = a->v_stride_l;
     p.o = (uint16_t*)a->o; p.o_sb = a->o_stride_b; p.o_sl = a->o_stride_l;
     p.bias = a->key_bias; p.bias_sb = a->bias_stride_b;
+    p.valid_keys = a->valid_keys;
+    LTXMI_REQUIRE((((uintptr_t)a->valid_keys) & 3) == 0, LTXMI_ERR_INVALID_ARG, "ltxmi_attention_fwd_bf16: valid_keys must be 4-byte aligned");
     p.B = a->B; p.H = a->H; p.Lq = a->Lq; p.Lk = a->Lk;
     p.scale_log2e = a->softmax_scale * LOG2E;
     p.q_tiles = (a->Lq + Q_PER_WG - 1) / Q_PER_WG;
@@ -446,7 +449,8 @@
                           LTXMI_ERR_INVALID_ARG, "ltxmi_attention_fwd_bf16: RoPE tables must be 16-byte aligned rows");
     }
     hipStream_t s = (hipStream_t)stream;
-    switch (attn_select(a->B, a->H, a->Lq, a->Lk, a->head_dim, a->key_bias != nullptr, a->k_stride_l, a->v_stride_l)) {
+    const bool has_bias = a->key_bias != nullptr || a->valid_keys != nullptr;
+    switch (attn_select(a->B, a->H, a->Lq, a->Lk, a->head_dim, has_bias, a->k_stride_l, a->v_stride_l)) {
         case ATTN_DH64: return launch<64, false, 1>(p, s);
         case ATTN_DH64_BIAS: return launch<64, true, 1>(p, s);
         case ATTN_DH64_QB2: return launch<64, false, ATTN_QB_BIG>(p, s);
diff --git a/ltx-video-gpupoor_amd/csrc/attention_cross.hip b/ltx-video-gpupoor_amd/csrc/attention_cross.hip
--- a/ltx-video-gpupoor_amd/csrc/attention_cross.hip
+++ b/ltx-video-gpupoor_amd/csrc/attention_cross.hip
@@ -26,28 +26,19 @@
 __device__ __forceinline__ int k_swz(int row) { return (row >> 1) & 7; }
 
 template <int NT>
-__global__ __launch_bounds__(256, 2) void attn_cross_kernel(AttnParams p, int groups, int rows_per_group, int stagger_from) {
+__device__ __forceinline__ void cross_slice(const AttnParams& p, int b, int head, int row_begin, int row_end, int lk, int stagger_from) {
     extern __shared__ __attribute__((aligned(16))) char smem[];
-    const int tid = threadIdx.x;
+    int tid = threadIdx.x;
+    asm volatile("" : "+v"(tid));
     const int lane = tid & 63;
     const int wave = __builtin_amdgcn_readfirstlane(tid >> 6);
     const int r = lane & 31, hh = lane >> 5;
-
-    const int nwg = gridDim.x, orig = blockIdx.x;
-    const int xcd = orig & 7, qn = nwg >> 3, rn = nwg & 7;
-    const int work = (xcd < rn ? xcd * (qn + 1) : rn * (qn + 1) + (xcd - rn) * qn) + (orig >> 3);
-    const int bh = work / groups, grp = work % groups;
-    const int b = bh / p.H, head = bh % p.H;
-    const int row_begin = grp * rows_per_group;
-    const int row_end = min(p.Lq, row_begin + rows_per_group);
-    if (row_begin >= row_end) return;
     const int n_it = (row_end - row_begin + ROWS_PER_IT - 1) / ROWS_PER_IT;
 
     const uint16_t* qb = p.q + (int64_t)b * p.q_sb + head * DH;
     const uint16_t* kb_ = p.k + (int64_t)b * p.k_sb + head * DH;
     const uint16_t* vb = p.v + (int64_t)b * p.v_sb + head * DH;
     uint16_t* ob = p.o + (int64_t)b * p.o_sb + head * DH;
-    constexpr int nt = NT;
 
     {
         u32x4 kreg[NT][2], vreg[NT][2];
@@ -64,7 +55,7 @@
             }
         if (tid < MAX_TILES * KV_TILE) {
             float bv = ATTN_BIAS_FLOOR;
-            if (tid < p.Lk) bv = p.bias ? fmaxf(p.bias[(int64_t)b * p.bias_sb + tid] * (LOG2E / p.scale_log2e), ATTN_BIAS_FLOOR) : 0.f;
+            if (tid < lk) bv = p.bias ? fmaxf(p.bias[(int64_t)b * p.bias_sb + tid] * (LOG2E / p.scale_log2e), ATTN_BIAS_FLOOR) : 0.f;
             const __bf16 hi = (__bf16)bv;
             const __bf16 lo = (__bf16)(bv - (float)hi);
             u32x4 w = {0u, 0u, 0u, 0u};
@@ -266,6 +257,31 @@
             }
         }
     }
+}
+
+template <int NT>
+__global__ __launch_bounds__(256, 2) void attn_cross_kernel(AttnParams p, int groups, int rows_per_group, int stagger_from) {
+    const int nwg = gridDim.x, orig = blockIdx.x;
+    const int xcd = orig & 7, qn = nwg >> 3, rn = nwg & 7;
+    const int work = (xcd < rn ? xcd * (qn + 1) : rn * (qn + 1) + (xcd - rn) * qn) + (orig >> 3);
+    const int bh = work / groups, grp = work % groups;
+    const int b = bh / p.H, head = bh % p.H;
+    const int row_begin = grp * rows_per_group;
+    const int row_end = min(p.Lq, row_begin + rows_per_group);
+    if (row_begin >= row_end) return;
+    int lk = p.Lk;
+    if (p.valid_keys != nullptr) lk = min(max(p.valid_keys[b], 1), p.Lk);
+    const int nt = __builtin_amdgcn_readfirstlane((lk + KV_TILE - 1) / KV_TILE);
+    if constexpr (NT > 1) {
+        if (nt == 1) return cross_slice<1>(p, b, head, row_begin, row_end, lk, stagger_from);
+    }
+    if constexpr (NT > 2) {
+        if (nt == 2) return cross_slice<2>(p, b, head, row_begin, row_end, lk, stagger_from);
+    }
+    if constexpr (NT > 3) {
+        if (nt == 3) return cross_slice<3>(p, b, head, row_begin, row_end, lk, stagger_from);
+    }
+    cross_slice<NT>(p, b, head, row_begin, row_end, lk, stagger_from);
 }
 
 }
diff --git a/ltx-video-gpupoor_amd/ltxmi/_lib.py b/ltx-video-gpupoor_amd/ltxmi/_lib.py
--- a/ltx-video-gpupoor_amd/ltxmi/_lib.py
+++ b/ltx-video-gpupoor_amd/ltxmi/_lib.py
@@ -23,7 +23,7 @@
                 ("k", c_void_p), ("k_stride_b", c_int64), ("k_stride_l", c_int64),
                 ("v", c_void_p), ("v_stride_b", c_int64), ("v_stride_l", c_int64),
                 ("o", c_void_p), ("o_stride_b", c_int64), ("o_stride_l", c_int64),
-                ("key_bias", c_void_p), ("bias_stride_b", c_int64),
+                ("key_bias", c_void_p), ("bias_stride_b", c_int64), ("valid_keys", c_void_p),
                 ("B", c_int), ("H", c_int), ("Lq", c_int), ("Lk", c_int), ("head_dim", c_int),
                 ("softmax_scale", c_float),
                 ("q_rowsumsq", c_void_p), ("q_rowsumsq_stride_b", c_int64), ("q_rowsumsq_stride_l", c_int64),
diff --git a/ltx-video-gpupoor_amd/ltxmi/attention.py b/ltx-video-gpupoor_amd/ltxmi/attention.py
--- a/ltx-video-gpupoor_amd/ltxmi/attention.py
+++ b/ltx-video-gpupoor_amd/ltxmi/attention.py
@@ -158,6 +158,16 @@
         return self.processor(self, wrapper, freqs_cis=freqs_cis, encoder_hidden_states=encoder_hidden_states,
                               attention_mask=attention_mask, skip_layer_mask=skip_layer_mask,
                               skip_layer_strategy=skip_layer_strategy, fused_residual=fused_residual)
+
+
+def _rows_of(ehs, full, full_version):
+    row_bytes = full.stride(0) * full.element_size()
+    off = ehs.data_ptr() - full.data_ptr()
+    if (row_bytes > 0 and off >= 0 and off % row_bytes == 0 and ehs.shape[1:] == full.shape[1:]
+            and off // row_bytes + ehs.shape[0] <= full.shape[0] and ehs.dtype == full.dtype and ehs.is_contiguous()
+            and ops.tensor_version(full) == full_version):
+        return off // row_bytes
+    return None
 
 
 def _host_mask(mask):
@@ -234,12 +244,8 @@
                 ready = attn.__dict__.get("_text_kv_ready")
                 if ready is not None:
                     full, full_version, kv_full = ready
-                    row_bytes = full.stride(0) * full.element_size()
-                    off = ehs.data_ptr() - full.data_ptr()
-                    if (row_bytes > 0 and off >= 0 and off % row_bytes == 0 and ehs.shape[1:] == full.shape[1:]
-                            and off // row_bytes + Bk <= full.shape[0] and ehs.dtype == full.dtype and ehs.is_contiguous()
-                            and ops.tensor_version(full) == full_version):
-                        r0 = off // row_bytes
+                    r0 = _rows_of(ehs, full, full_version)
+                    if r0 is not None:
                         hit = (kv_full[r0 * Lk:(r0 + Bk) * Lk],)
             if hit is None:
                 kv = ops.gemm(ehs.reshape(Bk * Lk, -1), wkv, bkv)
@@ -266,12 +272,19 @@
             a3 = v3.contiguous()
         else:
             mask4 = None
+            extra = {}
+            counts = attn.__dict__.get("_text_valid_keys") if is_cross and attention_mask is not None else None
+            if counts is not None:
+                full, full_version, vk_full = counts
+                r0 = _rows_of(encoder_hidden_states, full, full_version)
+                if r0 is not None and Bk == B:
+                    extra["valid_keys"] = vk_full[r0:r0 + Bk]
             if attention_mask is not None:
                 if attention_mask.dim() != 3 or attention_mask.shape[1] != 1:
                     raise NotImplementedError("ltxmi.AttnProcessor2_0: attention_mask must be a [B,1,Lk] bias")
                 mask4 = attention_mask.reshape(B, 1, 1, Lk)
             a4 = self.attend([q4, k4, v4], is_cross, attention_mask=mask4, softmax_scale=attn.scale,
-                             q_norm=q_fused[0] if q_fused else None, rope=q_fused[1] if q_fused else None)
+                             q_norm=q_fused[0] if q_fused else None, rope=q_fused[1] if q_fused else None, **extra)
             a3 = a4.view(B, N, D)
             if host_mask is not None and any(m != 1.0 for m in host_mask):
                 m_dev = skip_layer_mask.reshape(B).to(torch.float32)
diff --git a/ltx-video-gpupoor_amd/ltxmi/attention_seam.py b/ltx-video-gpupoor_amd/ltxmi/attention_seam.py
--- a/ltx-video-gpupoor_amd/ltxmi/attention_seam.py
+++ b/ltx-video-gpupoor_amd/ltxmi/attention_seam.py
@@ -27,11 +27,13 @@
 @torch.compiler.disable()
 def pay_attention(qkv_list, dropout_p=0., softmax_scale=None, causal=False, window_size=(-1, -1),
                   deterministic=False, version=None, force_attention=None, attention_mask=None,
-                  cross_attn=False, q_lens=None, k_lens=None, q_norm=None, rope=None):
+                  cross_attn=False, q_lens=None, k_lens=None, q_norm=None, rope=None, valid_keys=None):
     q, k, v = qkv_list
     qkv_list.clear()
     if (q_norm is not None or rope is not None) and (q_lens is not None or k_lens is not None):
         raise NotImplementedError("pay_attention: q_norm / rope on load with q_lens / k_lens")
+    if valid_keys is not None and (q_lens is not None or k_lens is not None):
+        raise NotImplementedError("pay_attention: valid_keys with q_lens / k_lens")
     if causal or tuple(window_size) != (-1, -1) or dropout_p != 0.:
         raise NotImplementedError("pay_attention: causal / windowed / dropout attention is not on this path")
     if force_attention not in (None, "sdpa"):
@@ -72,7 +74,8 @@
         q, k, v = q[:, :szq], k[:, :szk], v[:, :szk]
 
     bias = None if attention_mask is None else _key_bias_from_mask(attention_mask, b, k.size(1))
-    x = ops.attention(q, k, v, key_bias=bias, softmax_scale=softmax_scale, q_norm=q_norm, rope=rope)
+    extra = {} if valid_keys is None else {"valid_keys": valid_keys}
+    x = ops.attention(q, k, v, key_bias=bias, softmax_scale=softmax_scale, q_norm=q_norm, rope=rope, **extra)
     x = x.type(out_dtype)
     if final_padding > 0:
         x = torch.cat([x, torch.empty((x.shape[0], final_padding, *x.shape[-2:]), dtype=x.dtype, device=x.device)], 1)
diff --git a/ltx-video-gpupoor_amd/ltxmi/ops.py b/ltx-video-gpupoor_amd/ltxmi/ops.py
--- a/ltx-video-gpupoor_amd/ltxmi/ops.py
+++ b/ltx-video-gpupoor_amd/ltxmi/ops.py
@@ -186,7 +186,7 @@
 
 
 def attention(q, k, v, out=None, key_bias=None, softmax_scale=None, q_norm=None, rope=None, out_segments=None,
-              redo_counter=None, force_exact=False, return_lse=False, lse=None):
+              redo_counter=None, force_exact=False, return_lse=False, lse=None, valid_keys=None):
     _chk_bf16(q, k, v, out)
     B, Lq, H, dh = q.shape
     Lk = k.shape[1]
@@ -216,6 +216,10 @@
         if key_bias.dtype != torch.float32 or key_bias.shape != (B, Lk) or key_bias.stride(1) != 1:
             raise ValueError("ltxmi.attention: key_bias must be fp32 [B, Lk]")
         a.key_bias, a.bias_stride_b = key_bias.data_ptr(), key_bias.stride(0)
+    if valid_keys is not None:
+        if valid_keys.dtype != torch.int32 or tuple(valid_keys.shape) != (B,) or valid_keys.stride(0) != 1 or not valid_keys.is_cuda:
+            raise ValueError("ltxmi.attention: valid_keys must be a contiguous CUDA int32 [B]")
+        a.valid_keys = valid_keys.data_ptr()
     a.B, a.H, a.Lq, a.Lk, a.head_dim = B, H, Lq, Lk, dh
     a.softmax_scale = softmax_scale if softmax_scale is not None else 1.0 / math.sqrt(dh)
     if q_norm is not None:
@@ -517,6 +521,7 @@
 
 STEP_INVARIANT_CACHING = True
 STACKED_TEXT_KV = True
+CROSS_VALID_KEYS = True
 
 
 def set_step_invariant_caching(enabled: bool):
diff --git a/ltx-video-gpupoor_amd/ltxmi/transformer3d.py b/ltx-video-gpupoor_amd/ltxmi/transformer3d.py
--- a/ltx-video-gpupoor_amd/ltxmi/transformer3d.py
+++ b/ltx-video-gpupoor_amd/ltxmi/transformer3d.py
@@ -172,6 +172,27 @@
             sin_freq = torch.cat([torch.zeros_like(cos_freq[:, :, : dim % 6]), sin_freq], dim=-1)
         return cos_freq.to(self.dtype).contiguous(), sin_freq.to(self.dtype).contiguous()
 
+    def _drop_text_handover(self):
+        for block in self.transformer_blocks:
+            attn2 = getattr(block, "attn2", None)
+            if attn2 is not None:
+                attn2.__dict__.pop("_text_kv_ready", None)
+                attn2.__dict__.pop("_text_valid_keys", None)
+
+    @staticmethod
+    def _valid_text_keys(mask):
+        T = mask.shape[1]
+        pos = torch.arange(1, T + 1, device=mask.device, dtype=torch.int32)
+        last = ((mask != 0) * pos).amax(dim=1)
+        return torch.where(last == 0, T, last)
+
+    def _hand_over_valid_keys(self, ehs, valid_keys):
+        if valid_keys is None or ehs is None or ehs.dim() != 3 or not ehs.is_contiguous() or valid_keys.shape[0] != ehs.shape[0]:
+            return
+        for b in self.transformer_blocks:
+            if getattr(b, "attn2", None) is not None:
+                b.attn2.__dict__["_text_valid_keys"] = (ehs, ops.tensor_version(ehs), valid_keys)
+
     def _stacked_text_kv(self, ehs):
         blocks = [b for b in self.transformer_blocks if getattr(b, "attn2", None) is not None]
         if not blocks or ehs.dim() != 3 or not ehs.is_contiguous():
@@ -253,7 +274,11 @@
         B, N, _ = hidden_states.shape
         D = self.inner_dim
 
+        self._drop_text_handover()
+        valid_keys = None
         if encoder_attention_mask is not None and encoder_attention_mask.ndim == 2:
+            if ops.CROSS_VALID_KEYS and encoder_attention_mask.is_cuda:
+                valid_keys = self._valid_text_keys(encoder_attention_mask.to(dtype))
             encoder_attention_mask = ((1 - encoder_attention_mask.to(dtype)) * -10000.0).unsqueeze(1)
 
         hidden_states = ops.gemm(hidden_states.reshape(B * N, -1), self.patchify_proj.weight,
@@ -285,6 +310,8 @@
 
         if joint_pass and ops.STACKED_TEXT_KV and not ops.STEP_INVARIANT_CACHING and encoder_hidden_states is not None:
             self._stacked_text_kv(encoder_hidden_states)
+        if joint_pass:
+            self._hand_over_valid_keys(encoder_hidden_states, valid_keys)
 
         host_rows = None
         if skip_layer_mask is not None:
@@ -300,57 +327,57 @@
             m._ltxmi_host = rows if sl is None else rows[sl]
             return m
 
-        first_block = 0
-        if joint_pass and stg_alias_blocks and B >= 2:
-            heads, dh = self.num_attention_heads, self.attention_head_dim
-            if ops.attention_kernel_id(B, heads, N, N, dh) != ops.attention_kernel_id(B - 1, heads, N, N, dh):
-                stg_alias_blocks = 0
-        if joint_pass and stg_alias_blocks and B >= 2:
-            first_block = min(int(stg_alias_blocks), len(self.transformer_blocks))
-            keep = slice(0, B - 1)
-            hs = hidden_states[keep]
-            for block_idx in range(first_block):
-                self.transformer_blocks[block_idx](
-                    hs, freqs_cis=freqs_cis, attention_mask=attention_mask,
-                    encoder_hidden_states=encoder_hidden_states[keep],
-                    encoder_attention_mask=None if encoder_attention_mask is None else encoder_attention_mask[keep],
-                    timestep=temb[keep], cross_attention_kwargs=cross_attention_kwargs, class_labels=class_labels,
-                    skip_layer_mask=layer_mask(block_idx, keep), skip_layer_strategy=skip_layer_strategy)
-                if ltxv_model is not None and ltxv_model._interrupt:
-                    return [None]
-            hidden_states[B - 1].copy_(hidden_states[B - 2])
-        if joint_pass and _microbatches and len(_microbatches) > 1 and first_block == 0:
-            if self._run_blocks_microbatched(hidden_states, _microbatches, freqs_cis, attention_mask, encoder_hidden_states,
-                                             encoder_attention_mask, temb, cross_attention_kwargs, class_labels,
-                                             layer_mask, skip_layer_strategy, ltxv_model):
-                return [None]
-        elif joint_pass:
-            for block_idx, block in enumerate(self.transformer_blocks):
-                if block_idx < first_block:
-                    continue
-                hidden_states = block(hidden_states, freqs_cis=freqs_cis, attention_mask=attention_mask,
-                                      encoder_hidden_states=encoder_hidden_states,
-                                      encoder_attention_mask=encoder_attention_mask, timestep=temb,
-                                      cross_attention_kwargs=cross_attention_kwargs, class_labels=class_labels,
-                                      skip_layer_mask=layer_mask(block_idx),
-                                      skip_layer_strategy=skip_layer_strategy)
-                if ltxv_model is not None and ltxv_model._interrupt:
-                    return [None]
-        else:
-            for block_idx, block in enumerate(self.transformer_blocks):
-                for i in range(B):
-                    block(hidden_states[i:i + 1], freqs_cis=freqs_cis, attention_mask=attention_mask,
-                          encoder_hidden_states=encoder_hidden_states[i:i + 1],
-                          encoder_attention_mask=encoder_attention_mask[i:i + 1], timestep=temb[i:i + 1],
-                          cross_attention_kwargs=cross_attention_kwargs, class_labels=class_labels,
-                          skip_layer_mask=layer_mask(block_idx, slice(i, i + 1)),
-                          skip_layer_strategy=skip_layer_strategy)
+        try:
+            first_block = 0
+            if joint_pass and stg_alias_blocks and B >= 2:
+                heads, dh = self.num_attention_heads, self.attention_head_dim
+                if ops.attention_kernel_id(B, heads, N, N, dh) != ops.attention_kernel_id(B - 1, heads, N, N, dh):
+                    stg_alias_blocks = 0
+            if joint_pass and stg_alias_blocks and B >= 2:
+                first_block = min(int(stg_alias_blocks), len(self.transformer_blocks))
+                keep = slice(0, B - 1)
+                hs = hidden_states[keep]
+                for block_idx in range(first_block):
+                    self.transformer_blocks[block_idx](
+                        hs, freqs_cis=freqs_cis, attention_mask=attention_mask,
+                        encoder_hidden_states=encoder_hidden_states[keep],
+                        encoder_attention_mask=None if encoder_attention_mask is None else encoder_attention_mask[keep],
+                        timestep=temb[keep], cross_attention_kwargs=cross_attention_kwargs, class_labels=class_labels,
+                        skip_layer_mask=layer_mask(block_idx, keep), skip_layer_strategy=skip_layer_strategy)
                     if ltxv_model is not None and ltxv_model._interrupt:
                         return [None]
-
-        for block in self.transformer_blocks:
-            if getattr(block, "attn2", None) is not None:
-                block.attn2.__dict__.pop("_text_kv_ready", None)
+                hidden_states[B - 1].copy_(hidden_states[B - 2])
+            if joint_pass and _microbatches and len(_microbatches) > 1 and first_block == 0:
+                if self._run_blocks_microbatched(hidden_states, _microbatches, freqs_cis, attention_mask, encoder_hidden_states,
+                                                 encoder_attention_mask, temb, cross_attention_kwargs, class_labels,
+                                                 layer_mask, skip_layer_strategy, ltxv_model):
+                    return [None]
+            elif joint_pass:
+                for block_idx, block in enumerate(self.transformer_blocks):
+                    if block_idx < first_block:
+                        continue
+                    hidden_states = block(hidden_states, freqs_cis=freqs_cis, attention_mask=attention_mask,
+                                          encoder_hidden_states=encoder_hidden_states,
+                                          encoder_attention_mask=encoder_attention_mask, timestep=temb,
+                                          cross_attention_kwargs=cross_attention_kwargs, class_labels=class_labels,
+                                          skip_layer_mask=layer_mask(block_idx),
+                                          skip_layer_strategy=skip_layer_strategy)
+                    if ltxv_model is not None and ltxv_model._interrupt:
+                        return [None]
+            else:
+                for block_idx, block in enumerate(self.transformer_blocks):
+                    for i in range(B):
+                        block(hidden_states[i:i + 1], freqs_cis=freqs_cis, attention_mask=attention_mask,
+                              encoder_hidden_states=encoder_hidden_states[i:i + 1],
+                              encoder_attention_mask=encoder_attention_mask[i:i + 1], timestep=temb[i:i + 1],
+                              cross_attention_kwargs=cross_attention_kwargs, class_labels=class_labels,
+                              skip_layer_mask=layer_mask(block_idx, slice(i, i + 1)),
+                              skip_layer_strategy=skip_layer_strategy)
+                        if ltxv_model is not None and ltxv_model._interrupt:
+                            return [None]
+
+        finally:
+            self._drop_text_handover()
 
         T1 = embedded_timestep.shape[1]
         emb2 = embedded_timestep.reshape(B * T1, D)
```

Result: no change. 16.51, median of 6 (+0.8%).
